# ghnmqdtg/VM-ASR

Measured on AMD Instinct MI355X. Metric: audio clips/sec (train step) 48kHz n_fft=1024, higher is better.
Workload: dtype bf16 (autocast over G; scan/STFT f32; MPD f32/bf16x3 MFMA); 1 GPU; vm_asr_48k_MPD.yaml full train step, DIMS 16 d_state 1 n_fft 1024 clip 122640@48k; per_gpu_batch=4, global_batch=4, parallelism=dp1, execution=hipGraph replay, 2 streams, generator_streams=2

## Files before the change

### include/vmasr_hip.h

```cpp
#ifndef VMASR_HIP_H
#define VMASR_HIP_H

#include <stddef.h>
#include <stdint.h>

#ifdef __cplusplus
extern "C" {
#endif

#define VMASR_ABI_VERSION 1

typedef void *vmasr_stream_t;

enum { VMASR_F32 = 0, VMASR_F16 = 1, VMASR_BF16 = 2 };

enum {
    VMASR_OK = 0,
    VMASR_EINVAL = -1,
    VMASR_EALIGN = -2,
    VMASR_ENOSPACE = -3
};

int vmasr_abi_version(void);
const char *vmasr_last_error(void);
// ... 119 lines not shown
                           int32_t in_features, int32_t out_features, int32_t x_dtype, int32_t y_dtype,
                           vmasr_stream_t stream);
size_t vmasr_small_linear_bwd_workspace(int64_t rows, int32_t in_features, int32_t out_features);
int vmasr_small_linear_bwd(const void *x, const float *w, const void *gy, void *dx, float *dw, float *db,
                           float *ws, int64_t rows, int32_t in_features, int32_t out_features,
                           int32_t x_dtype, int32_t gy_dtype, vmasr_stream_t stream);

int vmasr_spectral_power_iter(const float *W, float *u, float *v, float *ws, int32_t R, int32_t C,
                              int32_t n_iter, float eps, vmasr_stream_t stream);

typedef struct vmasr_spectral_item {
    const float *W;
    float *u, *v, *t, *s;
    int32_t R, C, row_block_start, col_tile_start;
} vmasr_spectral_item;
int vmasr_spectral_power_iter_batched(const vmasr_spectral_item *items, int32_t n, int32_t total_row_blocks,
                                      int32_t total_col_tiles, int64_t weight_bytes, int32_t n_iter, float eps,
                                      float *sigma, vmasr_stream_t stream);

int vmasr_im2col_kx1(const void *x, void *cols, int64_t N, int32_t H, int32_t C, int32_t k, int32_t stride,
                     int32_t pad, int64_t rows_out, int32_t dtype, vmasr_stream_t stream);
int vmasr_im2col_kx1_split(const float *x, void *hi, void *lo, int64_t N, int32_t H, int32_t C, int32_t k, int32_t stride,
                           int32_t pad, int64_t rows_out, vmasr_stream_t stream);
int vmasr_col2im_kx1(const void *dcols, void *dx, int64_t N, int32_t H, int32_t C, int32_t k, int32_t stride,
                     int32_t pad, int32_t dtype, vmasr_stream_t stream);
int vmasr_im2col_kx1_split_multi(const float *const *xs, const int64_t *Ns, const int32_t *Hs, int32_t n, void *hi, void *lo,
                                 int32_t C, int32_t k, int32_t stride, int32_t pad, int64_t rows_out, vmasr_stream_t stream);
int vmasr_im2col_kx1_split3_multi(const float *const *xs, const int64_t *Ns, const int32_t *Hs, int32_t n, void *cat3, int32_t C,
                                  int32_t k, int32_t stride, int32_t pad, int64_t rows_out, vmasr_stream_t stream);
int vmasr_col2im_kx1_multi(const void *dcols, void *const *dxs, const int64_t *Ns, const int32_t *Hs, int32_t n, int32_t C,
                           int32_t k, int32_t stride, int32_t pad, int64_t rows, int32_t dtype, vmasr_stream_t stream);
int vmasr_col2im_kx1_stacked(const void *dcols, void *dx, const int64_t *Ns, const int32_t *Hs, int32_t n, int32_t C, int32_t k, int32_t stride,
                             int32_t pad, int64_t rows, int64_t dx_rows, int32_t dtype, vmasr_stream_t stream);
int vmasr_stack_rows(const void *const *srcs, const int64_t *Ms, int32_t n, void *full, int64_t rows, int64_t row_bytes,
                     vmasr_stream_t stream);


int vmasr_bias_gelu_fwd(float *acc, const float *bias, float *act, int32_t slots, int64_t M, int32_t N, int32_t parts,
                        vmasr_stream_t stream);
int vmasr_weight_prep_split(const float *w, void *out, int32_t n, int32_t N, int32_t K, vmasr_stream_t stream);
int vmasr_weight_transpose(const float *w, void *hi, void *lo, float *out32, int32_t n, int32_t N, int32_t Cin, int32_t k,
                           vmasr_stream_t stream);
int vmasr_sum_parts(const float *parts, float *out, int32_t P, int32_t n, int32_t S, int64_t NK, vmasr_stream_t stream);
int vmasr_gelu_bwd_split(const float *pre, const float *g, void *hi, void *lo, void *cat3, float *db, int32_t slots, int64_t M,
                         int32_t N, vmasr_stream_t stream);
int vmasr_gelu_bwd(const float *pre, const float *g, float *gx, float *db, int32_t slots, int64_t M, int32_t N, vmasr_stream_t stream);

typedef struct vmasr_cg_slot {
    const void *ah, *al;
    const void *bh, *bl;
    float *c0;
    float *c1;
    void *ch, *cl;
    const float *bias;
    int64_t nseq;
    int32_t H;
    int32_t reserved;
} vmasr_cg_slot;
int vmasr_conv_mfma_supported(int32_t Cin, int32_t Cout, int32_t k, int32_t stride);
int vmasr_conv_mfma_supported_launch(int32_t Cin, int32_t Cout, int32_t k, int32_t stride, int32_t n, int64_t rows);
int vmasr_conv_mfma_config(int32_t pass, int32_t Cin, int32_t Cout, int32_t ops, int32_t out[3]);
void vmasr_conv_set_cu_limit(int32_t cus);
int32_t vmasr_conv_get_cu_limit(void);
int vmasr_conv_mfma_fwd(const vmasr_cg_slot *slots, int32_t n, int32_t Cin, int32_t Cout, int32_t k, int32_t stride, int32_t pad,
                        int64_t rows_out, int32_t act, vmasr_stream_t stream);
int vmasr_conv_mfma_dgrad(const vmasr_cg_slot *slots, int32_t n, int32_t Cin, int32_t Cout, int32_t k, int32_t stride, int32_t pad,
                          int64_t rows_in, vmasr_stream_t stream);
int vmasr_conv_f32_fwd(const vmasr_cg_slot *slots, int32_t n, int32_t Cin, int32_t Cout, int32_t k, int32_t stride, int32_t pad,
                       int64_t rows_out, int32_t act, vmasr_stream_t stream);
int vmasr_conv_f32_dgrad(const vmasr_cg_slot *slots, int32_t n, int32_t Cin, int32_t Cout, int32_t k, int32_t stride, int32_t pad,
                         int64_t rows_in, vmasr_stream_t stream);
int vmasr_conv_mfma_wgrad(const vmasr_cg_slot *slots, int32_t n, int32_t Cin, int32_t Cout, int32_t k, int32_t stride, int32_t pad,
                          int32_t splits, vmasr_stream_t stream);
typedef struct vmasr_cg_gelu_bwd {
    const float *pre;
    const signed char *sgn;
    int64_t valid;
    float scale;
    int32_t reserved;
    float *db;
} vmasr_cg_gelu_bwd;
int vmasr_conv_mfma_dgrad_gelu(const vmasr_cg_slot *slots, const vmasr_cg_gelu_bwd *epi, const float *gtok, int32_t n, int32_t Cin, int32_t Cout,
                               int32_t k, int32_t stride, int32_t pad, int64_t rows_in, vmasr_stream_t stream);

int vmasr_wgrad_finish_multi(const float *const *parts, float *const *dws, float *const *dbs, float *const *e1s, float *const *e2s,
                             const int32_t *Ss, const int32_t *Ns, const int32_t *Ks, const int32_t *lds, int32_t n, vmasr_stream_t stream);

int vmasr_linear_f64acc(const float *x, const float *w, const float *bias, float *y, int64_t rows, int32_t out_features,
                        int32_t in_features, vmasr_stream_t stream);

typedef struct vmasr_adamw_item {
    float *p;
    const float *g;
    float *m;
    float *v;
    void *lp;
    int64_t n;
    float weight_decay;
    int32_t vec;
    void *lpt;
    int32_t rows, cols;
} vmasr_adamw_item;
int32_t vmasr_adamw_chunk(void);
int vmasr_adamw_step(const vmasr_adamw_item *items, const int32_t *chunks, int32_t nchunks, int64_t total_elems, const float *lr,
                     const float *step, float beta1, float beta2, float eps, vmasr_stream_t stream);

int32_t vmasr_sn_dot_blocks(void);
int vmasr_sn_stack_fwd(const void *const *weights, const void *const *sigmas, int32_t n, float *out, void *hi, void *lo, int32_t N, int32_t Cin,
                       int32_t k, vmasr_stream_t stream);
int vmasr_sn_stack_bwd(const float *dW, const float *Wn, void *const *gws, const void *const *sigmas, const void *const *us,
                       const void *const *vs, int32_t n, double *partials, int32_t N, int32_t Cin, int32_t k, vmasr_stream_t stream);

int vmasr_conv_post_supported(int32_t C, int32_t k);
int vmasr_conv_post_fwd(const float *x, const float *w, const float *b, float *y, const int64_t *Ms, const int32_t *Hs, int32_t n, int64_t rows,
                        int32_t C, int32_t k, vmasr_stream_t stream);
int vmasr_conv_post_bwd(const float *x, const float *w, const float *gy, float *dx, float *dw, float *db, const int64_t *Ms, const int32_t *Hs,
                        int32_t n, int64_t rows, int32_t C, int32_t k, vmasr_stream_t stream);
int vmasr_conv_post_bwd_gelu(const float *x, const float *w, const float *gy, const float *pre, const void *sgn, const float *gtok,
                             const int64_t *valid, const float *scale, void *gh, void *gl, float *g32, float *dw, float *db, float *dbcol,
                             const int64_t *Ms, const int32_t *Hs, int32_t n, int64_t rows, int32_t C, int32_t k, vmasr_stream_t stream);

int vmasr_conv_first_fwd(const void *const *xs, const int64_t *Ns, const int32_t *Hs, int32_t n, const float *w, const float *b, float *pre,
                         float *act, int64_t rows, vmasr_stream_t stream);
int vmasr_conv_first_bwd(const void *const *xs, const int64_t *Ns, const int32_t *Hs, int32_t n, const float *w, const float *pre,
                         const float *g, float *dcols, float *dw, float *db, int64_t rows, vmasr_stream_t stream);

int32_t vmasr_masked_l1_blocks(void);
int vmasr_masked_l1_fwd(const float *real, const float *gen, void *sgn, double *partials, const int64_t *valid, const float *scale,
                        int32_t n, int64_t rows_r, int64_t rows_g, int32_t N, vmasr_stream_t stream);
int vmasr_masked_l1_bwd(const void *sgn, const float *gout, float *dgen, const int64_t *valid, const float *scale, int32_t n,
                        int64_t rows_g, int32_t N, vmasr_stream_t stream);
int vmasr_masked_l1_bwd_add(const void *sgn, const float *gout, const float *add, float *dgen, const int64_t *valid, const float *scale,
                            int32_t n, int64_t rows_g, int32_t N, vmasr_stream_t stream);
int vmasr_lsgan_fwd(const void *const *xs, const int64_t *ns, const float *targets, int32_t count, float *out, vmasr_stream_t stream);
int vmasr_lsgan_bwd(const void *const *xs, void *const *ds, const int64_t *ns, const float *targets, int32_t count, const float *gout,
                    vmasr_stream_t stream);

#define VMASR_SS2D_PAIRS 1
typedef struct vmasr_ss2d_params {
    int32_t B, D, H, W, dtype, flags;
    const void *x;
    void *xT;
    const float *Wx, *Wdt, *dtb, *Alog, *Ds;
    float *state, *out02, *out13, *y;
    const float *dy;
    float *dyT, *adj, *part;
    void *dx;
    float *dWx, *dWdt, *ddtb, *dAlog, *dDs;
} vmasr_ss2d_params;
int vmasr_ss2d_supported(int32_t d_state, int32_t dt_rank, int32_t d_inner, int32_t H, int32_t W);
size_t vmasr_ss2d_part_floats(int32_t B, int32_t D, int32_t H, int32_t W);
int vmasr_ss2d_fwd(const vmasr_ss2d_params *p, vmasr_stream_t stream);
int vmasr_ss2d_bwd(const vmasr_ss2d_params *p, vmasr_stream_t stream);

typedef struct vmasr_ss2d_deep_params {
    int32_t B, D, H, W, R, dtype;
    const void *x;
    const float *WxT, *Wdt, *dtb, *Alog, *Ds;
    float *xdbl, *y;
    const float *dy;
    float *du;
    void *tp, *tb, *tc;
    float *pg, *g32;
    void *dx, *gpos;
} vmasr_ss2d_deep_params;
int vmasr_ss2d_deep_supported(int32_t d_state, int32_t dt_rank, int32_t d_inner, int32_t H, int32_t W);
// ... 97 lines not shown
int vmasr_dconv1d_dgrad(const float *gy, const float *pre, const float *w, float *dx, void *ws, size_t ws_bytes, int32_t B, int32_t Cin,
                        int32_t Cout, int32_t groups, int64_t L, int32_t k, int32_t stride, int32_t pad, vmasr_stream_t stream);
int vmasr_dconv1d_wgrad(const float *x, const float *gy, const float *pre, float *dw, float *db, void *ws, size_t ws_bytes, int32_t B,
                        int32_t Cin, int32_t Cout, int32_t groups, int64_t L, int32_t k, int32_t stride, int32_t pad, vmasr_stream_t stream);

enum {
    VMASR_K_SSCAN_FWD = 0,
    VMASR_K_SSCAN_FWD_AGG,
    VMASR_K_SSCAN_FWD_CARRY,
    VMASR_K_SSCAN_FWD_APPLY,
    VMASR_K_SSCAN_BWD,
    VMASR_K_SSCAN_BWD_AGG,
    VMASR_K_SSCAN_BWD_CARRY,
    VMASR_K_SSCAN_BWD_APPLY,
    VMASR_K_CROSS_SCAN,
    VMASR_K_CROSS_MERGE,
    VMASR_K_DWCONV_FWD,
    VMASR_K_DWCONV_BWD_A,
    VMASR_K_DWCONV_BWD_B,
    VMASR_K_STFT,
    VMASR_K_ISTFT_FRAMES,
    VMASR_K_ISTFT_OLA,
    VMASR_K_ISTFT_BWD,
    VMASR_K_LN_FWD,
    VMASR_K_LN_BWD,
    VMASR_K_LN_BWD_REDUCE,
    VMASR_K_SMALL_LINEAR_FWD,
    VMASR_K_SMALL_LINEAR_BWD,
    VMASR_K_SMALL_LINEAR_REDUCE,
    VMASR_K_XPROJ_FWD,
    VMASR_K_XPROJ_BWD_A,
    VMASR_K_XPROJ_BWD_B,
    VMASR_K_SPECTRAL,
    VMASR_K_IM2COL,
    VMASR_K_COL2IM,
    VMASR_K_SPLIT_BF16,
    VMASR_K_BIAS_GELU,
    VMASR_K_SS2D_TRANSPOSE,
    VMASR_K_SS2D_FWD_AGG,
    VMASR_K_SS2D_CARRY,
    VMASR_K_SS2D_FWD_APPLY,
    VMASR_K_SS2D_MERGE,
    VMASR_K_SS2D_BWD_AGG,
    VMASR_K_SS2D_BWD_APPLY,
    VMASR_K_SS2D_PRE,
    VMASR_K_LN_GATE,
    VMASR_K_STACK_ROWS,
    VMASR_K_FEAT_L1,
    VMASR_K_ADAMW,
    VMASR_K_CONV_POST,
    VMASR_K_CONV_POST_BWD_GELU,
    VMASR_K_WEIGHT_T,
    VMASR_K_MLP_FWD,
    VMASR_K_MLP_BWD,
    VMASR_K_INPROJ_FWD,
    VMASR_K_INPROJ_BWD,
    VMASR_K_SS2D_DEEP_XPROJ,
    VMASR_K_SS2D_DEEP_FWD,
    VMASR_K_SS2D_DEEP_BWD,
    VMASR_K_SS2D_DEEP_XBWD,
    VMASR_K_OUTPROJ_FWD,
    VMASR_K_OUTPROJ_BWD,
    VMASR_K_STFT_LOSS,
    VMASR_K_CONV_MFMA_FWD,
    VMASR_K_CONV_MFMA_DGRAD,
    VMASR_K_CONV_MFMA_WGRAD,
    VMASR_K_WGRAD_FINISH,
    VMASR_K_SKINNY_LINEAR,
    VMASR_K_METRICS,
    VMASR_K_RESAMPLE_DESIGN,
    VMASR_K_DEGRADE_BATCH,
    VMASR_K_GCONV1D_FWD,
    VMASR_K_GCONV1D_DGRAD,
    VMASR_K_GCONV1D_WGRAD,
    VMASR_K_GCONV1D_WGRAD_REDUCE,
    VMASR_K_STEM1D_FWD,
    VMASR_K_STEM1D_BWD,
    VMASR_K_STEM1D_BWD_REDUCE,
    VMASR_K_DCONV1D_FWD,
    VMASR_K_DCONV1D_DGRAD,
    VMASR_K_DCONV1D_REDUCE,
    VMASR_K_DCONV1D_WGRAD,
    VMASR_K_DCONV1D_WGRAD_REDUCE,
    VMASR_K_RESAMPLE,
    VMASR_K_COUNT
};
void vmasr_set_deterministic(int on);
int vmasr_get_deterministic(void);
int64_t vmasr_det_timeouts(void);
void vmasr_prof_enable(int on);
void vmasr_prof_reset(void);
const char *vmasr_prof_name(int kernel_id);
int vmasr_prof_collect(int kernel_id, int64_t *launches, double *total_ms, double *alg_bytes);
int vmasr_mark_time(uint64_t *dst, vmasr_stream_t stream);

int vmasr_im2col2d_rows(const void *x, void *cols, int32_t B, int32_t C, int32_t H, int32_t W, int32_t kh, int32_t kw, int32_t sh, int32_t sw,
                        int32_t ph, int32_t pw, const int64_t *x_strides, int32_t x_dtype, int32_t cols_dtype, vmasr_stream_t stream);
int vmasr_col2im2d_rows(const void *gcols, void *dx, int32_t B, int32_t C, int32_t H, int32_t W, int32_t kh, int32_t kw, int32_t sh, int32_t sw,
                        int32_t ph, int32_t pw, const int64_t *dx_strides, int32_t cols_dtype, int32_t dx_dtype, vmasr_stream_t stream);
int vmasr_skinny_linear_supported(int64_t rows, int32_t in_f, int32_t out_f);
int vmasr_skinny_linear(const void *x, const float *w, const float *bias, void *y, int64_t rows, int32_t in_f, int32_t out_f,
                        int64_t w_stride_out, int64_t w_stride_in, int32_t x_dtype, int32_t y_dtype, vmasr_stream_t stream);
int vmasr_prof_collect_shapes(int kernel_id, int max_groups, double *group_bytes, int64_t *group_launches, double *group_ms);

#ifdef __cplusplus
}
#endif
#endif
```

### vm_asr_amd/_lib.py

```python
import ctypes
import os

from . import knobs

_HERE = os.path.dirname(os.path.abspath(__file__))
LIB_PATH = knobs.get("VMASR_LIB") or os.path.join(_HERE, "libvmasr_hip.so")

c_i32, c_i64, c_vp, c_sz = ctypes.c_int32, ctypes.c_int64, ctypes.c_void_p, ctypes.c_size_t

F32, F16, BF16 = 0, 1, 2


class SScanParams(ctypes.Structure):
    _fields_ = (
        [(n, c_i32) for n in ("batch", "dim", "seqlen", "dstate", "n_groups", "n_chunks", "dtype",
                              "delta_softplus")]
        + [(n, c_i64) for n in ("A_d_stride", "A_dstate_stride",
                                "B_batch_stride", "B_group_stride", "B_dstate_stride",
                                "C_batch_stride", "C_group_stride", "C_dstate_stride",
                                "u_batch_stride", "u_d_stride", "delta_batch_stride", "delta_d_stride",
                                "out_batch_stride", "out_d_stride")]
        + [(n, c_vp) for n in ("A_ptr", "B_ptr", "C_ptr", "D_ptr", "u_ptr", "delta_ptr",
                               "delta_bias_ptr", "out_ptr", "x_ptr")]
    )


class SScanBwdParams(ctypes.Structure):
    _fields_ = (
        [("f", SScanParams)]
        + [(n, c_i64) for n in ("dout_batch_stride", "dout_d_stride", "du_batch_stride", "du_d_stride",
                                "ddelta_batch_stride", "ddelta_d_stride", "dA_d_stride", "dA_dstate_stride")]
        + [(n, c_vp) for n in ("dout_ptr", "du_ptr", "ddelta_ptr", "dA_ptr", "dB_ptr", "dC_ptr", "dD_ptr",
                               "ddelta_bias_ptr", "ws_ptr")]
        + [("ws_bytes", c_sz)]
    )


class SS2DParams(ctypes.Structure):
    _fields_ = ([(n, c_i32) for n in ("B", "D", "H", "W", "dtype", "flags")]
                + [(n, c_vp) for n in ("x", "xT", "Wx", "Wdt", "dtb", "Alog", "Ds", "state", "out02", "out13", "y",
                                       "dy", "dyT", "adj", "part", "dx", "dWx", "dWdt", "ddtb", "dAlog", "dDs")])


class CgSlot(ctypes.Structure):
    _fields_ = ([(n, c_vp) for n in ("ah", "al", "bh", "bl", "c0", "c1", "ch", "cl", "bias")]
                + [("nseq", c_i64), ("H", c_i32), ("reserved", c_i32)])


class CgGeluBwd(ctypes.Structure):
    _fields_ = [("pre", c_vp), ("sgn", c_vp), ("valid", c_i64), ("scale", ctypes.c_float), ("reserved", c_i32), ("db", c_vp)]


class SS2DDeepParams(ctypes.Structure):
    _fields_ = ([(n, c_i32) for n in ("B", "D", "H", "W", "R", "dtype")]
                + [(n, c_vp) for n in ("x", "WxT", "Wdt", "dtb", "Alog", "Ds", "xdbl", "y", "dy", "du", "tp", "tb", "tc", "pg",
                                       "g32", "dx", "gpos")])


SYMBOLS = {
    "vmasr_abi_version": (ctypes.c_int, []),
    "vmasr_last_error": (ctypes.c_char_p, []),
    "vmasr_sscan_chunk": (ctypes.c_int, []),
    "vmasr_sscan_fwd": (ctypes.c_int, [ctypes.POINTER(SScanParams), c_vp]),
    "vmasr_sscan_bwd_workspace": (c_sz, [ctypes.POINTER(SScanBwdParams)]),
    "vmasr_sscan_bwd": (ctypes.c_int, [ctypes.POINTER(SScanBwdParams), c_vp]),
    "vmasr_sscan_tune": (None, [ctypes.c_int, ctypes.c_int]),
    "vmasr_layer_norm_fwd": (ctypes.c_int, [c_vp, c_vp, c_vp, c_vp, c_vp, c_vp, c_i32, c_i32, ctypes.c_float, c_i32, c_i32, c_vp]),
    "vmasr_layer_norm_bwd_workspace": (c_sz, [c_i32, c_i32]),
    "vmasr_layer_norm_bwd": (ctypes.c_int, [c_vp, c_vp, c_vp, c_vp, c_vp, c_vp, c_vp, c_vp, c_vp, c_i32, c_i32, c_i32, c_i32, c_vp]),
    "vmasr_layer_norm_bwd_res": (ctypes.c_int, [c_vp, c_vp, c_vp, c_vp, c_vp, c_vp, c_vp, c_vp, c_vp, c_vp, c_i32, c_i32, c_i32, c_i32, c_vp]),
    "vmasr_layer_norm_bwd_blocks": (c_i32, [c_i32, c_i32]),
    "vmasr_layer_norm_bwd_reduce_multi": (ctypes.c_int, [c_vp, c_vp, c_vp, c_vp, c_vp, c_i32, c_vp]),
    "vmasr_mlp_supported": (ctypes.c_int, [c_i32, c_i32]),
    "vmasr_mlp_fwd": (ctypes.c_int, [c_vp, c_vp, c_vp, ctypes.c_float, c_vp, c_vp, c_vp, c_vp, c_vp, c_i32, c_vp, c_i64, c_i32, c_i32, c_vp]),
    "vmasr_mlp_bwd": (ctypes.c_int, [c_vp, c_vp, c_vp, c_vp, ctypes.c_float, c_vp, c_vp, c_vp, c_vp, c_vp, c_i32,
                                     c_vp, c_vp, c_vp, c_vp, c_vp, c_vp, c_vp, c_i64, c_i32, c_i32, c_vp]),
    "vmasr_stft_loss_blocks": (c_i32, []),
    "vmasr_stft_loss_fwd": (ctypes.c_int, [c_vp, c_vp, c_vp, c_vp, c_i64, c_vp, c_vp, c_vp]),
    "vmasr_stft_loss_bwd": (ctypes.c_int, [c_vp, c_vp, c_vp, c_vp, c_i64, c_vp, c_vp, c_vp, c_vp, c_vp, c_vp]),
    "vmasr_outproj_supported": (ctypes.c_int, [c_i32, c_i32]),
    "vmasr_outproj_fwd": (ctypes.c_int, [c_vp, c_vp, c_vp, c_vp, c_i32, c_vp, c_i64, c_i32, c_i32, c_vp]),
    "vmasr_outproj_bwd": (ctypes.c_int, [c_vp, c_vp, c_vp, c_i32, c_vp, c_vp, c_i64, c_i32, c_i32, c_vp]),
    "vmasr_inproj_supported": (ctypes.c_int, [c_i32, c_i32, c_i64]),
    "vmasr_inproj_fwd": (ctypes.c_int, [c_vp, c_vp, c_vp, ctypes.c_float, c_vp, c_vp, c_vp, c_i64, c_i32, c_i32, c_i32, c_vp]),
    "vmasr_inproj_bwd": (ctypes.c_int, [c_vp, c_vp, c_vp, ctypes.c_float, c_vp, c_vp, c_vp, c_vp, c_vp, c_vp, c_vp, c_vp, c_vp,
                                        c_i64, c_i32, c_i32, c_i32, c_vp]),
    "vmasr_small_linear_supported": (ctypes.c_int, [c_i32, c_i32]),
    "vmasr_small_linear_fwd": (ctypes.c_int, [c_vp, c_vp, c_vp, c_vp, c_i64, c_i32, c_i32, c_i32, c_i32, c_vp]),
    "vmasr_small_linear_bwd_workspace": (c_sz, [c_i64, c_i32, c_i32]),
    "vmasr_small_linear_bwd": (ctypes.c_int, [c_vp, c_vp, c_vp, c_vp, c_vp, c_vp, c_vp, c_i64, c_i32, c_i32, c_i32, c_i32, c_vp]),
    "vmasr_cross_scan_cvt": (ctypes.c_int, [c_vp, c_vp, c_i32, c_i32, c_i32, c_i32, c_i32, c_i32, c_vp]),
    "vmasr_cross_merge_cvt": (ctypes.c_int, [c_vp, c_vp, c_i32, c_i32, c_i32, c_i32, c_i32, c_i32, c_vp]),
    "vmasr_xproj_supported": (ctypes.c_int, [c_i32, c_i32, c_i32]),
    "vmasr_xproj_fwd": (ctypes.c_int, [c_vp] * 7 + [c_i32] * 7 + [c_vp]),
    "vmasr_xproj_bwd": (ctypes.c_int, [c_vp] * 12 + [c_i32] * 7 + [c_vp]),
    "vmasr_xproj_n_supported": (ctypes.c_int, [c_i32, c_i32, c_i32]),
    "vmasr_xproj_n_ws_floats": (c_sz, [c_i32, c_i32, c_i32, c_i32]),
    "vmasr_xproj_n_fwd": (ctypes.c_int, [c_vp] * 7 + [c_i32] * 7 + [c_vp]),
    "vmasr_xproj_n_bwd": (ctypes.c_int, [c_vp] * 12 + [c_i32] * 7 + [c_vp]),
    "vmasr_spectral_power_iter": (ctypes.c_int, [c_vp, c_vp, c_vp, c_vp, c_i32, c_i32, c_i32, ctypes.c_float, c_vp]),
    "vmasr_spectral_power_iter_batched": (ctypes.c_int, [c_vp, c_i32, c_i32, c_i32, c_i64, c_i32, ctypes.c_float, c_vp, c_vp]),
    "vmasr_im2col_kx1": (ctypes.c_int, [c_vp, c_vp, c_i64, c_i32, c_i32, c_i32, c_i32, c_i32, c_i64, c_i32, c_vp]),
    "vmasr_im2col_kx1_split": (ctypes.c_int, [c_vp, c_vp, c_vp, c_i64, c_i32, c_i32, c_i32, c_i32, c_i32, c_i64, c_vp]),
    "vmasr_im2col_kx1_split3_multi": (ctypes.c_int, [c_vp, c_vp, c_vp, c_i32, c_vp, c_i32, c_i32, c_i32, c_i32, c_i64, c_vp]),
    "vmasr_col2im_kx1": (ctypes.c_int, [c_vp, c_vp, c_i64, c_i32, c_i32, c_i32, c_i32, c_i32, c_i32, c_vp]),
    "vmasr_im2col_kx1_split_multi": (ctypes.c_int, [c_vp, c_vp, c_vp, c_i32, c_vp, c_vp, c_i32, c_i32, c_i32, c_i32, c_i64, c_vp]),
    "vmasr_col2im_kx1_multi": (ctypes.c_int, [c_vp, c_vp, c_vp, c_vp, c_i32, c_i32, c_i32, c_i32, c_i32, c_i64, c_i32, c_vp]),
    "vmasr_col2im_kx1_stacked": (ctypes.c_int, [c_vp, c_vp, c_vp, c_vp, c_i32, c_i32, c_i32, c_i32, c_i32, c_i64, c_i64, c_i32, c_vp]),
    "vmasr_stack_rows": (ctypes.c_int, [c_vp, c_vp, c_i32, c_vp, c_i64, c_i64, c_vp]),
    "vmasr_split_bf16": (ctypes.c_int, [c_vp, c_vp, c_vp, c_i64, c_vp]),
    "vmasr_bias_gelu_fwd": (ctypes.c_int, [c_vp, c_vp, c_vp, c_i32, c_i64, c_i32, c_i32, c_vp]),
    "vmasr_gelu_bwd": (ctypes.c_int, [c_vp, c_vp, c_vp, c_vp, c_i32, c_i64, c_i32, c_vp]),
    "vmasr_sn_dot_blocks": (c_i32, []),
    "vmasr_sn_stack_fwd": (ctypes.c_int, [c_vp, c_vp, c_i32, c_vp, c_vp, c_vp, c_i32, c_i32, c_i32, c_vp]),
    "vmasr_sn_stack_bwd": (ctypes.c_int, [c_vp, c_vp, c_vp, c_vp, c_vp, c_vp, c_i32, c_vp, c_i32, c_i32, c_i32, c_vp]),
    "vmasr_conv_post_supported": (ctypes.c_int, [c_i32, c_i32]),
    "vmasr_conv_post_fwd": (ctypes.c_int, [c_vp, c_vp, c_vp, c_vp, c_vp, c_vp, c_i32, c_i64, c_i32, c_i32, c_vp]),
    "vmasr_conv_post_bwd": (ctypes.c_int, [c_vp, c_vp, c_vp, c_vp, c_vp, c_vp, c_vp, c_vp, c_i32, c_i64, c_i32, c_i32, c_vp]),
    "vmasr_conv_post_bwd_gelu": (ctypes.c_int, [c_vp] * 16 + [c_i32, c_i64, c_i32, c_i32, c_vp]),
    "vmasr_conv_first_fwd": (ctypes.c_int, [c_vp, c_vp, c_vp, c_i32, c_vp, c_vp, c_vp, c_vp, c_i64, c_vp]),
    "vmasr_conv_first_bwd": (ctypes.c_int, [c_vp, c_vp, c_vp, c_i32, c_vp, c_vp, c_vp, c_vp, c_vp, c_vp, c_i64, c_vp]),
    "vmasr_adamw_chunk": (c_i32, []),
    "vmasr_adamw_step": (ctypes.c_int, [c_vp, c_vp, c_i32, c_i64, c_vp, c_vp, ctypes.c_float, ctypes.c_float, ctypes.c_float, c_vp]),
    "vmasr_masked_l1_blocks": (c_i32, []),
    "vmasr_masked_l1_fwd": (ctypes.c_int, [c_vp, c_vp, c_vp, c_vp, c_vp, c_vp, c_i32, c_i64, c_i64, c_i32, c_vp]),
    "vmasr_masked_l1_bwd": (ctypes.c_int, [c_vp, c_vp, c_vp, c_vp, c_vp, c_i32, c_i64, c_i32, c_vp]),
    "vmasr_lsgan_fwd": (ctypes.c_int, [c_vp, c_vp, c_vp, c_i32, c_vp, c_vp]),
    "vmasr_lsgan_bwd": (ctypes.c_int, [c_vp, c_vp, c_vp, c_vp, c_i32, c_vp, c_vp]),
    "vmasr_masked_l1_bwd_add": (ctypes.c_int, [c_vp, c_vp, c_vp, c_vp, c_vp, c_vp, c_i32, c_i64, c_i32, c_vp]),
    "vmasr_sum_parts": (ctypes.c_int, [c_vp, c_vp, c_i32, c_i32, c_i32, c_i64, c_vp]),
    "vmasr_weight_prep_split": (ctypes.c_int, [c_vp, c_vp, c_i32, c_i32, c_i32, c_vp]),
    "vmasr_weight_transpose": (ctypes.c_int, [c_vp, c_vp, c_vp, c_vp, c_i32, c_i32, c_i32, c_i32, c_vp]),
    "vmasr_gelu_bwd_split": (ctypes.c_int, [c_vp, c_vp, c_vp, c_vp, c_vp, c_vp, c_i32, c_i64, c_i32, c_vp]),
    "vmasr_conv_mfma_supported": (ctypes.c_int, [c_i32, c_i32, c_i32, c_i32]),
    "vmasr_conv_mfma_supported_launch": (ctypes.c_int, [c_i32, c_i32, c_i32, c_i32, c_i32, ctypes.c_int64]),
    "vmasr_conv_mfma_config": (ctypes.c_int, [c_i32, c_i32, c_i32, c_i32, ctypes.POINTER(c_i32)]),
    "vmasr_mark_time": (ctypes.c_int, [c_vp, c_vp]),
    "vmasr_im2col2d_rows": (ctypes.c_int, [c_vp, c_vp] + [c_i32] * 10 + [c_vp, c_i32, c_i32, c_vp]),
    "vmasr_col2im2d_rows": (ctypes.c_int, [c_vp, c_vp] + [c_i32] * 10 + [c_vp, c_i32, c_i32, c_vp]),
    "vmasr_skinny_linear_supported": (ctypes.c_int, [c_i64, c_i32, c_i32]),
    "vmasr_skinny_linear": (ctypes.c_int, [c_vp, c_vp, c_vp, c_vp, c_i64, c_i32, c_i32, c_i64, c_i64, c_i32, c_i32, c_vp]),
    "vmasr_conv_set_cu_limit": (None, [c_i32]),
    "vmasr_conv_get_cu_limit": (c_i32, []),
    "vmasr_conv_mfma_fwd": (ctypes.c_int, [ctypes.POINTER(CgSlot), c_i32, c_i32, c_i32, c_i32, c_i32, c_i32, c_i64, c_i32, c_vp]),
    "vmasr_conv_mfma_dgrad": (ctypes.c_int, [ctypes.POINTER(CgSlot), c_i32, c_i32, c_i32, c_i32, c_i32, c_i32, c_i64, c_vp]),
    "vmasr_conv_f32_fwd": (ctypes.c_int, [ctypes.POINTER(CgSlot), c_i32, c_i32, c_i32, c_i32, c_i32, c_i32, c_i64, c_i32, c_vp]),
    "vmasr_conv_f32_dgrad": (ctypes.c_int, [ctypes.POINTER(CgSlot), c_i32, c_i32, c_i32, c_i32, c_i32, c_i32, c_i64, c_vp]),
    "vmasr_conv_mfma_wgrad": (ctypes.c_int, [ctypes.POINTER(CgSlot), c_i32, c_i32, c_i32, c_i32, c_i32, c_i32, c_i32, c_vp]),
    "vmasr_conv_mfma_dgrad_gelu": (ctypes.c_int, [ctypes.POINTER(CgSlot), ctypes.POINTER(CgGeluBwd), c_vp, c_i32, c_i32, c_i32, c_i32, c_i32,
                                                  c_i32, c_i64, c_vp]),
    "vmasr_wgrad_finish_multi": (ctypes.c_int, [c_vp, c_vp, c_vp, c_vp, c_vp, c_vp, c_vp, c_vp, c_vp, c_i32, c_vp]),
    "vmasr_linear_f64acc": (ctypes.c_int, [c_vp, c_vp, c_vp, c_vp, c_i64, c_i32, c_i32, c_vp]),
    "vmasr_ss2d_glue_supported": (ctypes.c_int, [c_i32, c_i32, c_i32]),
    "vmasr_ss2d_pre_fwd": (ctypes.c_int, [c_vp, c_vp, c_vp, c_i32, c_i32, c_i32, c_i32, c_vp]),
    "vmasr_ss2d_pre_bwd": (ctypes.c_int, [c_vp, c_vp, c_vp, c_vp, c_i32, c_i32, c_i32, c_i32, c_vp]),
    "vmasr_ln_gate_fwd": (ctypes.c_int, [c_vp] * 7 + [c_i32, c_i32, c_i32, ctypes.c_float, c_i32, c_vp]),
    "vmasr_ln_gate_bwd": (ctypes.c_int, [c_vp] * 11 + [c_i32, c_i32, c_i32, c_i32, c_vp]),
    "vmasr_ln_gate_bwd_workspace": (c_i64, [c_i32, c_i32, c_i32, c_i32]),
    "vmasr_ln_gate_bwd_ws": (ctypes.c_int, [c_vp] * 12 + [c_i32, c_i32, c_i32, c_i32, c_vp]),
    "vmasr_ln_gate_pair_supported": (ctypes.c_int, [c_i32, c_i32, c_i32]),
    "vmasr_ln_gate_pair_fwd": (ctypes.c_int, [c_vp] * 8 + [c_i32, c_i32, c_i32, c_i32, ctypes.c_float, c_i32, c_vp]),
    "vmasr_ln_gate_pair_bwd": (ctypes.c_int, [c_vp] * 13 + [c_i32, c_i32, c_i32, c_i32, c_i32, c_vp]),
    "vmasr_ss2d_supported": (ctypes.c_int, [c_i32] * 5),
    "vmasr_ss2d_part_floats": (c_sz, [c_i32] * 4),
    "vmasr_ss2d_fwd": (ctypes.c_int, [ctypes.POINTER(SS2DParams), c_vp]),
    "vmasr_ss2d_bwd": (ctypes.c_int, [ctypes.POINTER(SS2DParams), c_vp]),
    "vmasr_ss2d_deep_supported": (ctypes.c_int, [c_i32] * 5),
    "vmasr_ss2d_deep_waves_per_row": (c_i32, [c_i32, c_i32]),
    "vmasr_ss2d_deep_fwd": (ctypes.c_int, [ctypes.POINTER(SS2DDeepParams), c_vp]),
    "vmasr_ss2d_deep_bwd": (ctypes.c_int, [ctypes.POINTER(SS2DDeepParams), c_vp]),
    "vmasr_set_deterministic": (None, [ctypes.c_int]),
    "vmasr_get_deterministic": (ctypes.c_int, []),
    "vmasr_det_timeouts": (ctypes.c_int64, []),
    "vmasr_prof_enable": (None, [ctypes.c_int]),
    "vmasr_prof_reset": (None, []),
    "vmasr_prof_name": (ctypes.c_char_p, [ctypes.c_int]),
    "vmasr_prof_collect": (ctypes.c_int, [ctypes.c_int, ctypes.POINTER(ctypes.c_int64),
                                          ctypes.POINTER(ctypes.c_double), ctypes.POINTER(ctypes.c_double)]),
    "vmasr_prof_collect_shapes": (ctypes.c_int, [ctypes.c_int, ctypes.c_int, ctypes.POINTER(ctypes.c_double), ctypes.POINTER(ctypes.c_int64),
                                                 ctypes.POINTER(ctypes.c_double)]),
    "vmasr_cross_scan": (ctypes.c_int, [c_vp, c_vp, c_i32, c_i32, c_i32, c_i32, c_i32, c_vp]),
    "vmasr_cross_merge": (ctypes.c_int, [c_vp, c_vp, c_i32, c_i32, c_i32, c_i32, c_i32, c_vp]),
    "vmasr_dwconv_silu_fwd": (ctypes.c_int, [c_vp, c_vp, c_vp, c_vp, c_i32, c_i32, c_i32, c_i32, c_i32, c_vp]),
    "vmasr_dwconv_silu_bwd": (ctypes.c_int, [c_vp, c_vp, c_vp, c_vp, c_vp, c_vp, c_vp, c_vp,
                                             c_i32, c_i32, c_i32, c_i32, c_i32, c_vp]),
    "vmasr_stft": (ctypes.c_int, [c_vp, c_vp, c_vp, c_i32, c_i32, c_i32, c_i32, c_i32, c_i32, c_i32, c_vp]),
    "vmasr_stft_bwd_workspace": (c_sz, [c_i32, c_i32, c_i32, c_i32]),
    "vmasr_stft_bwd": (ctypes.c_int, [c_vp, c_vp, c_vp, c_i32, c_i32, c_i32, c_i32, c_i32, c_i32, c_vp, c_sz, c_vp]),
    "vmasr_istft_workspace": (c_sz, [c_i32, c_i32, c_i32, c_i32]),
    "vmasr_istft": (ctypes.c_int, [c_vp, c_vp, c_vp, c_i32, c_i32, c_i32, c_i32, c_i32, c_vp, c_sz, c_vp]),
    "vmasr_istft_bwd": (ctypes.c_int, [c_vp, c_vp, c_vp, c_vp, c_vp, c_i32, c_i32, c_i32, c_i32, c_i32, c_vp]),
    "vmasr_metrics_workspace": (c_sz, [c_i32, c_i32, c_i32, c_i32]),
    "vmasr_metrics": (ctypes.c_int, [c_vp, c_vp, c_vp, c_vp, c_vp, c_i32, c_i32, c_i32, c_i32, c_vp, c_sz, c_vp]),
    "vmasr_gconv1d_supported": (ctypes.c_int, [c_i32] * 5),
    "vmasr_gconv1d_supported_launch": (ctypes.c_int, [c_i32] * 7 + [c_i64]),
    "vmasr_gconv1d_wgrad_workspace": (c_sz, [c_i32] * 7 + [c_i64]),
    "vmasr_gconv1d_fwd": (ctypes.c_int, [c_vp] * 5 + [c_i32] * 4 + [c_i64] + [c_i32] * 4 + [c_vp]),
    "vmasr_gconv1d_dgrad": (ctypes.c_int, [c_vp] * 4 + [c_i32] * 4 + [c_i64] + [c_i32] * 3 + [c_vp]),
    "vmasr_gconv1d_wgrad": (ctypes.c_int, [c_vp] * 6 + [c_sz] + [c_i32] * 4 + [c_i64] + [c_i32] * 3 + [c_vp]),
    "vmasr_dconv1d_pos_tile": (c_i32, []),
    "vmasr_dconv1d_m_tile": (c_i32, []),
    "vmasr_dconv1d_k_chunk": (c_i32, []),
    "vmasr_dconv1d_max_taps": (c_i32, []),
    "vmasr_dconv1d_supported": (ctypes.c_int, [c_i32] * 5),
    "vmasr_dconv1d_supported_launch": (ctypes.c_int, [c_i32] * 7 + [c_i64]),
    "vmasr_dconv1d_fwd_slabs": (c_i32, [c_i32] * 7 + [c_i64]),
    "vmasr_dconv1d_fwd_workspace": (c_sz, [c_i32] * 7 + [c_i64]),
    "vmasr_dconv1d_dgrad_workspace": (c_sz, [c_i32] * 7 + [c_i64]),
    "vmasr_dconv1d_wgrad_workspace": (c_sz, [c_i32] * 7 + [c_i64]),
    "vmasr_dconv1d_fwd": (ctypes.c_int, [c_vp] * 6 + [c_sz] + [c_i32] * 4 + [c_i64] + [c_i32] * 4 + [c_vp]),
    "vmasr_dconv1d_dgrad": (ctypes.c_int, [c_vp] * 5 + [c_sz] + [c_i32] * 4 + [c_i64] + [c_i32] * 3 + [c_vp]),
    "vmasr_dconv1d_wgrad": (ctypes.c_int, [c_vp] * 6 + [c_sz] + [c_i32] * 4 + [c_i64] + [c_i32] * 3 + [c_vp]),
    "vmasr_stem1d_time_tile": (c_i32, []),
    "vmasr_stem1d_channel_group": (c_i32, []),
    "vmasr_stem1d_supported": (ctypes.c_int, [c_i32] * 4),
    "vmasr_stem1d_supported_launch": (ctypes.c_int, [c_i32] * 5 + [c_i64]),
    "vmasr_stem1d_bwd_workspace": (c_sz, [c_i32] * 5 + [c_i64]),
    "vmasr_stem1d_fwd": (ctypes.c_int, [c_vp] * 4 + [c_i32] * 2 + [c_i64] + [c_i32] * 4 + [c_vp]),
    "vmasr_stem1d_bwd": (ctypes.c_int, [c_vp] * 8 + [c_sz] + [c_i32] * 2 + [c_i64] + [c_i32] * 4 + [c_vp]),
    "vmasr_stem1d_fm_supported_launch": (ctypes.c_int, [c_i32] * 5 + [c_i64]),
    "vmasr_stem1d_fm_workspace": (c_sz, [c_i32] * 5 + [c_i64]),
    "vmasr_stem1d_fm_fwd": (ctypes.c_int, [c_vp] * 6 + [c_sz] + [c_i32] * 2 + [c_i64] + [c_i32] * 3 + [c_vp]),
    "vmasr_stem1d_fm_bwd": (ctypes.c_int, [c_vp] * 6 + [ctypes.c_float] + [c_vp] + [c_i32] * 2 + [c_i64] + [c_i32] * 3 + [c_vp]),
    "vmasr_resample_poly": (ctypes.c_int, [c_vp, c_vp, c_vp, c_i32, c_i64, c_i64, c_i32, c_i32, c_i32, c_vp]),
    "vmasr_resample_design_workspace": (c_sz, [c_i32]),
    "vmasr_resample_design": (ctypes.c_int, [c_vp, c_i32, c_i32, c_i32, c_vp, c_sz, c_vp]),
    "vmasr_degrade_batch_workspace": (c_sz, [c_vp, c_i32]),
# ... 22 lines not shown
        knobs.warn_undeclared()
        _lib = l
    return _lib


def check(code, what):
    if code != 0:
        msg = lib().vmasr_last_error().decode() or "unknown error"
        raise RuntimeError(f"{what} failed ({code}): {msg}")


def torch_dtype_code(dt):
    import torch
    try:
        return {torch.float32: F32, torch.float16: F16, torch.bfloat16: BF16}[dt]
    except KeyError:
        raise RuntimeError(f"unsupported dtype {dt}: expected float32 / float16 / bfloat16")


def det_mode():
    if knobs.get("VMASR_DETERMINISTIC"):
        return True
    try:
        return bool(lib().vmasr_get_deterministic())
    except (OSError, RuntimeError, AttributeError):
        return False


def current_stream(device):
    import torch
    return ctypes.c_void_p(torch.cuda.current_stream(device).cuda_stream)


def ptr(t):
    return None if t is None else ctypes.c_void_p(t.data_ptr())


def call(fn, *args, device=None):
    import torch
    what = fn.__name__[len("vmasr_"):]
    conv = list(args)
    for i, a in enumerate(conv):
        t = type(a)
        if t is int or t is float or a is None:
            continue
        if isinstance(a, torch.Tensor):
            if not a.is_cuda:
                require_cuda(what, a)
            if device is None:
                device = a.device
            conv[i] = ctypes.c_void_p(a.data_ptr())
        elif isinstance(a, ctypes.Structure):
            conv[i] = ctypes.byref(a)
    if device is None:
        raise RuntimeError(f"{what}: no tensor argument and no device= to launch on")
    with torch.cuda.device(device):
        check(fn(*conv, current_stream(device)), what)


def require_cuda(name, *tensors):
    if not all(t.is_cuda for t in tensors):
        raise RuntimeError(f"{name}: expected a CUDA (HIP) tensor; vm_asr_amd has no CPU path")


def bf16_autocast():
    import torch
    return torch.is_autocast_enabled("cuda") and torch.get_autocast_dtype("cuda") == torch.bfloat16


def autocast_dtype(x):
    import torch
    return torch.get_autocast_dtype("cuda") if torch.is_autocast_enabled("cuda") else x.dtype


def f32c(t, shape):
    return t.detach().float().reshape(shape).contiguous()


def rows2d(t, width):
    t2 = t.reshape(-1, width)
    return t2 if t2.is_contiguous() else t2.contiguous()


K_COUNT = 78


def zeros_f32(device, *shapes):
    import torch
    sizes = [0 if sh is None else -(-int(torch.Size(sh).numel()) // 4) * 4 for sh in shapes]
    flat = torch.zeros(max(1, sum(sizes)), dtype=torch.float32, device=device)
    out, off = [], 0
    for sh, n in zip(shapes, sizes):
        out.append(None if sh is None else flat[off:off + torch.Size(sh).numel()].view(sh))
        off += n
    return out


def prof_enable(on=True):
    lib().vmasr_prof_enable(int(bool(on)))


def prof_reset():
    lib().vmasr_prof_reset()


def prof_collect():
    l = lib()
    out = {}
    for k in range(K_COUNT):
        n, ms, by = ctypes.c_int64(0), ctypes.c_double(0.0), ctypes.c_double(0.0)
        check(l.vmasr_prof_collect(k, ctypes.byref(n), ctypes.byref(ms), ctypes.byref(by)), "prof_collect")
        if n.value:
            out[l.vmasr_prof_name(k).decode()] = dict(launches=n.value, ms=ms.value, alg_bytes=by.value)
    return out


def prof_collect_shapes(name, max_groups=16):
    l = lib()
    for k in range(K_COUNT):
        if l.vmasr_prof_name(k).decode() == name:
            by, n, ms = (ctypes.c_double * max_groups)(), (ctypes.c_int64 * max_groups)(), (ctypes.c_double * max_groups)()
            ng = l.vmasr_prof_collect_shapes(k, max_groups, by, n, ms)
            if ng < 0:
                raise RuntimeError(f"prof_collect_shapes failed ({ng})")
            return [dict(alg_bytes_per_launch=by[i], launches=n[i], ms=ms[i]) for i in range(ng)]
    raise KeyError(name)
```

### vm_asr_amd/convgemm.py

```python
import ctypes

import torch

from . import _lib
from .mpd_ops import need as _need, sum_parts


def supported(Cin, Cout, k, stride):
    return bool(_lib.lib().vmasr_conv_mfma_supported(int(Cin), int(Cout), int(k), int(stride)))


def config(what, Cin, Cout, f32=False):
    out = (ctypes.c_int32 * 3)()
    _lib.check(_lib.lib().vmasr_conv_mfma_config(("fwd", "dgrad", "wgrad").index(what), int(Cin), int(Cout), int(bool(f32)), out), "conv_mfma_config")
    return tuple(out)


_LIMIT = {"cus": 0, "min_channels": 0}


class cu_limit:

    def __init__(self, cus, min_channels=0):
        self.new = {"cus": int(cus or 0), "min_channels": int(min_channels or 0)}

    def __enter__(self):
        self.prev = dict(_LIMIT)
        _LIMIT.update(self.new)
        return self

    def __exit__(self, *exc):
        _LIMIT.update(self.prev)
        _lib.lib().vmasr_conv_set_cu_limit(0)
        return False


def _apply_limit(Cin, Cout):
    lim = _LIMIT["cus"] if max(Cin, Cout) >= _LIMIT["min_channels"] else 0
    _lib.lib().vmasr_conv_set_cu_limit(lim)


def _slots(geom, **operands):
    sl = (_lib.CgSlot * len(geom))()
    steps = [(f, t.data_ptr(), t.stride(0) * t.element_size()) for f, t in operands.items() if t is not None]
    for i, (nseq, H) in enumerate(geom):
        for f, base, step in steps:
            setattr(sl[i], f, base + i * step)
        sl[i].nseq, sl[i].H = int(nseq), int(H)
    return sl


def _ptr(t, i, step):
    return ctypes.c_void_p(t.data_ptr() + i * step) if t is not None else None


def out_positions(H, k, stride, pad):
    return (H + 2 * pad - k) // stride + 1


def _fwd(fn, xh, xl, wh, wl, bias, geom, k, stride, pad, rows_out, act, want_pair):
    _need(xh, xl, wh, wl, bias)
    (n, _, Cin), Cout, dev = xh.shape, wh.shape[1], xh.device
    pre = torch.empty((n, rows_out, Cout), dtype=torch.float32, device=dev)
    y = torch.empty_like(pre) if act else None
    yh = torch.empty((n, rows_out, Cout), dtype=torch.bfloat16, device=dev) if act and want_pair else None
    yl = torch.empty_like(yh) if yh is not None else None
    sl = _slots(geom, ah=xh, al=xl, bh=wh, bl=wl, c0=pre, c1=y, ch=yh, cl=yl, bias=bias)
    _apply_limit(Cin, Cout)
    _lib.call(fn, sl, n, Cin, Cout, k, stride, pad, rows_out, int(bool(act)), device=dev)
    return pre, y, yh, yl


def _dgrad(fn, gh, gl, wth, wtl, geom, k, stride, pad, rows_in):
    _need(gh, gl, wth, wtl)
    (n, _, Cout), Cin, dev = gh.shape, wth.shape[1], gh.device
    dx = torch.empty((n, rows_in, Cin), dtype=torch.float32, device=dev)
    sl = _slots(geom, ah=gh, al=gl, bh=wth, bl=wtl, c0=dx)
    _apply_limit(Cin, Cout)
    _lib.call(fn, sl, n, Cin, Cout, k, stride, pad, rows_in, device=dev)
    return dx


def conv_fwd(xh, xl, wh, wl, bias, geom, k, stride, pad, rows_out, act=True, want_pair=True):
    return _fwd(_lib.lib().vmasr_conv_mfma_fwd, xh, xl, wh, wl, bias, geom, k, stride, pad, rows_out, act, want_pair)


def conv_dgrad(gh, gl, wth, wtl, geom, k, stride, pad, rows_in):
    return _dgrad(_lib.lib().vmasr_conv_mfma_dgrad, gh, gl, wth, wtl, geom, k, stride, pad, rows_in)


def conv_fwd_f32(x, w, bias, geom, k, stride, pad, rows_out, act=True, want_pair=True):
    assert x.dtype == torch.float32 and w.dtype == torch.float32
    return _fwd(_lib.lib().vmasr_conv_f32_fwd, x, None, w, None, bias, geom, k, stride, pad, rows_out, act, want_pair)


def conv_dgrad_f32(g, wt, geom, k, stride, pad, rows_in):
    assert g.dtype == torch.float32 and wt.dtype == torch.float32
    return _dgrad(_lib.lib().vmasr_conv_f32_dgrad, g, None, wt, None, geom, k, stride, pad, rows_in)


def conv_dgrad_gelu(gh, gl, wth, wtl, geom, k, stride, pad, rows_in, pre, want_f32=False, want_pair=True, sgn=None, gtok=None,
                    scale=None, valid=None, db=None):
    _need(gh, gl, wth, wtl, pre, sgn, gtok, db)
    assert db is None or (db.shape == (gh.shape[0], wth.shape[1]) and db.dtype == torch.float32)
    (n, _, Cout), Cin, dev = gh.shape, wth.shape[1], gh.device
    assert pre.shape == (n, rows_in, Cin) and pre.dtype == torch.float32 and (want_f32 or want_pair)
    assert sgn is None or (sgn.shape == pre.shape and sgn.dtype == torch.int8 and gtok is not None and gtok.dtype == torch.float32)
    g32 = torch.empty((n, rows_in, Cin), dtype=torch.float32, device=dev) if want_f32 else None
    oh = torch.empty((n, rows_in, Cin), dtype=torch.bfloat16, device=dev) if want_pair else None
    ol = torch.empty_like(oh) if want_pair else None
    sl = _slots(geom, ah=gh, al=gl, bh=wth, bl=wtl, c0=g32, ch=oh, cl=ol)
    ep = (_lib.CgGeluBwd * n)()
    for i in range(n):
        ep[i].pre = _ptr(pre, i, rows_in * Cin * 4)
        ep[i].sgn = _ptr(sgn, i, rows_in * Cin)
        ep[i].valid = int(valid[i]) if (sgn is not None and valid is not None) else 0
        ep[i].scale = float(scale[i]) if (sgn is not None and scale is not None) else 0.0
        ep[i].db = _ptr(db, i, Cin * 4)
    _apply_limit(Cin, Cout)
    _lib.call(_lib.lib().vmasr_conv_mfma_dgrad_gelu, sl, ep, gtok if sgn is not None else None, n, Cin, Cout, k, stride, pad, rows_in,
              device=dev)
    return g32, ((oh, ol) if want_pair else None)


def wgrad_splits(n, Cin, Cout, k, M):
    if Cin % 256 == 0 and Cout % 256 == 0:
        return 1
    T = 128
    tiles = n * (Cout // T) * (k * Cin // T)
    s = 1
    while tiles * s < 768 and s < 16 and M // (2 * s) >= 1024:
        s *= 2
    return s


def conv_wgrad(gh, gl, xh, xl, geom, k, stride, pad, splits=None):
    _need(gh, gl, xh, xl)
    (n, _, Cout), Cin, dev = gh.shape, xh.shape[2], gh.device
    if splits is None:
        M = max(nseq * out_positions(H, k, stride, pad) for nseq, H in geom)
        splits = wgrad_splits(n, Cin, Cout, k, M)
    parts = torch.empty((n, splits, Cout, k * Cin), dtype=torch.float32, device=dev)
    sl = _slots(geom, ah=gh, al=gl, bh=xh, bl=xl, c0=parts)
    _apply_limit(Cin, Cout)
    _lib.call(_lib.lib().vmasr_conv_mfma_wgrad, sl, n, Cin, Cout, k, stride, pad, splits, device=dev)
    if splits == 1:
        return parts.view(n, Cout, k * Cin)
    return sum_parts(parts, 1, n, splits, (Cout, k * Cin))
```

### vm_asr_amd/csrc/api.hip

```cpp
#include "common.h"

#include <mutex>
#include <vector>

namespace vmasr {
namespace {
thread_local char g_err[512] = "";

struct Rec {
    int kid;
    hipEvent_t e0, e1;
    double bytes;
};
std::mutex g_mu;
std::vector<Rec> g_recs;
std::vector<hipEvent_t> g_pool;
thread_local Rec g_open{-1, nullptr, nullptr, 0.0};

hipEvent_t take_event() {
    if (!g_pool.empty()) {
        hipEvent_t e = g_pool.back();
        g_pool.pop_back();
        return e;
    }
    hipEvent_t e = nullptr;
    (void)hipEventCreate(&e);
    return e;
}

const char *kNames[VMASR_K_COUNT] = {
    "sscan_fwd", "sscan_fwd_agg", "sscan_fwd_carry", "sscan_fwd_apply", "sscan_bwd", "sscan_bwd_agg",
    "sscan_bwd_carry", "sscan_bwd_apply", "cross_scan", "cross_merge", "dwconv_silu_fwd", "dwconv_silu_bwd_a",
    "dwconv_silu_bwd_b", "stft", "istft_frames", "istft_ola", "istft_bwd", "layer_norm_fwd", "layer_norm_bwd",
    "layer_norm_bwd_reduce", "small_linear_fwd", "small_linear_bwd", "small_linear_reduce",
    "xproj_fwd", "xproj_bwd_a", "xproj_bwd_b", "spectral_power_iter", "im2col_kx1", "col2im_kx1", "split_bf16", "bias_gelu",
    "ss2d_transpose", "ss2d_fwd_agg", "ss2d_carry", "ss2d_fwd_apply", "ss2d_merge", "ss2d_bwd_agg", "ss2d_bwd_apply",
    "ss2d_pre", "ln_gate", "stack_rows", "feat_l1", "adamw", "conv_post", "conv_post_bwd_gelu", "weight_transpose", "mlp_fwd", "mlp_bwd", "inproj_fwd", "inproj_bwd",
    "ss2d_deep_xproj", "ss2d_deep_fwd", "ss2d_deep_bwd", "ss2d_deep_xbwd", "outproj_fwd", "outproj_bwd", "stft_loss",
    "conv_mfma_fwd", "conv_mfma_dgrad", "conv_mfma_wgrad", "wgrad_finish", "skinny_linear", "metrics", "resample_design", "degrade_batch",
    "gconv1d_fwd", "gconv1d_dgrad", "gconv1d_wgrad", "gconv1d_wgrad_reduce",
    "stem1d_fwd", "stem1d_bwd", "stem1d_bwd_reduce",
    "dconv1d_fwd", "dconv1d_dgrad", "dconv1d_reduce", "dconv1d_wgrad", "dconv1d_wgrad_reduce", "resample_poly"};
}

bool g_prof_on = false;
static bool g_det_on = false;
constexpr int kMaxDev = 16;
static unsigned *g_det_buf[kMaxDev] = {};

unsigned *det_ticket(int kid) {
    if (!g_det_on || kid < 0 || kid >= VMASR_K_COUNT) return nullptr;
    int dev = 0;
    if (hipGetDevice(&dev) != hipSuccess || dev < 0 || dev >= kMaxDev || g_det_buf[dev] == nullptr) {
        set_error("deterministic mode: no ticket buffer for device %d (vmasr_set_deterministic(1) must run before the first launch)", dev);
        return nullptr;
    }
    return g_det_buf[dev] + kid;
}
static int det_prepare() {
    int n = 0, cur = 0;
    if (hipGetDeviceCount(&n) != hipSuccess || n <= 0) return 0;
    (void)hipGetDevice(&cur);
    int rc = 0;
    for (int d = 0; d < n && d < kMaxDev; ++d) {
        if (g_det_buf[d]) continue;
        if (hipSetDevice(d) != hipSuccess || hipMalloc(reinterpret_cast<void **>(&g_det_buf[d]), 2 * VMASR_K_COUNT * sizeof(unsigned)) != hipSuccess ||
            hipMemset(g_det_buf[d], 0, 2 * VMASR_K_COUNT * sizeof(unsigned)) != hipSuccess || hipDeviceSynchronize() != hipSuccess) {
            g_det_buf[d] = nullptr;
            set_error("deterministic mode: cannot allocate the ticket buffer of device %d (switch the mode on outside a stream capture)", d);
            rc = VMASR_EINVAL;
        }
    }
    (void)hipSetDevice(cur);
    return rc;
}
void det_set(bool on) { g_det_on = on; }
bool det_get() { return g_det_on; }

void set_error(const char *fmt, ...) {
    va_list ap;
    va_start(ap, fmt);
    vsnprintf(g_err, sizeof(g_err), fmt, ap);
    va_end(ap);
}

void prof_begin(int kid, hipStream_t st, double bytes) {
    std::lock_guard<std::mutex> lk(g_mu);
    g_open = Rec{kid, take_event(), take_event(), bytes};
    (void)hipEventRecord(g_open.e0, st);
}

void prof_end(hipStream_t st) {
    std::lock_guard<std::mutex> lk(g_mu);
    if (g_open.kid < 0) return;
    (void)hipEventRecord(g_open.e1, st);
    g_recs.push_back(g_open);
    g_open.kid = -1;
}
}

using namespace vmasr;

VMASR_EXPORT int vmasr_abi_version(void) { return VMASR_ABI_VERSION; }
VMASR_EXPORT const char *vmasr_last_error(void) { return g_err; }

VMASR_EXPORT void vmasr_prof_enable(int on) { g_prof_on = on != 0; }

VMASR_EXPORT void vmasr_set_deterministic(int on) {
    if (on && vmasr::det_prepare() != 0) return;
    vmasr::det_set(on != 0);
}
VMASR_EXPORT int64_t vmasr_det_timeouts(void) {
    int64_t total = 0;
    int cur = 0;
    (void)hipGetDevice(&cur);
    for (int d = 0; d < vmasr::kMaxDev; ++d) {
        if (!vmasr::g_det_buf[d]) continue;
        unsigned host[VMASR_K_COUNT];
        if (hipSetDevice(d) != hipSuccess || hipDeviceSynchronize() != hipSuccess ||
            hipMemcpy(host, vmasr::g_det_buf[d] + VMASR_K_COUNT, sizeof(host), hipMemcpyDeviceToHost) != hipSuccess) { total = -1; break; }
        for (unsigned v : host) total += v;
    }
    (void)hipSetDevice(cur);
    return total;
}
// ... 68 lines not shown
```

### vm_asr_amd/csrc/convgemm.hip

```cpp
#include <algorithm>
#include <cstdlib>
#include <type_traits>

#include "common.h"

namespace vmasr {
namespace {

typedef __bf16 bf16x8 __attribute__((ext_vector_type(8)));
typedef float f32x16 __attribute__((ext_vector_type(16)));
typedef float f32x4 __attribute__((ext_vector_type(4)));
typedef unsigned u32x4 __attribute__((ext_vector_type(4)));
typedef __attribute__((address_space(1))) const void *cg_gptr;
typedef __attribute__((address_space(3))) void *cg_lptr;
__device__ uint4 cg_zero_page[4];

constexpr int CG_BM = 128, CG_BN = 128, CG_BK = 32;
constexpr int CG_TILE = CG_BM * CG_BK * 2;
constexpr int CG_STAGE = 4 * CG_TILE;
constexpr int CG_MAXP = 24;

struct CgProb {
    const bf16_t *ah, *al, *bh, *bl;
    float *c0, *c1;
    bf16_t *ch, *cl;
    const float *bias;
    int M, Q;
    int HA;
    int HC;
    int hq_mul, hq_add;
    int crow_mul, crow_add;
    int ntaps, tap0, tap_step, dstep;
    int tile_start, mtiles;
    int zero_rows;
    float fscale;
    int fvalid;
    float *db;
};

struct CgParams {
    CgProb prob[CG_MAXP];
    int nprob, ntiles_n, total_tiles;
    int CA;
    int NB;
    int KB;
    const float *gtok;
};
static_assert(sizeof(CgParams) <= 4096, "CgParams is passed by value as the kernel's argument block");

__device__ __forceinline__ int cg_swz(const int row) { return (0 - (row >> 2)) & 3; }
__device__ __forceinline__ int cg_off(const int row, const int chunk) { return row * 64 + ((chunk ^ cg_swz(row)) << 4); }

__device__ __forceinline__ float cg_gelu(float x) { return 0.5f * x * (1.f + erff(x * 0.70710678118654752f)); }
__device__ __forceinline__ float cg_gelu_grad(float x) {
    return 0.5f * (1.f + erff(x * 0.70710678118654752f)) + x * 0.3989422804014327f * __expf(-0.5f * x * x);
}

__device__ __forceinline__ f32x16 cg_mfma(const bf16x8 a, const bf16x8 b, const f32x16 c) {
    return __builtin_amdgcn_mfma_f32_32x32x16_bf16(a, b, c, 0, 0, 0);
}

template <int BM, int BN, int WM, int WN, int EPI, int MF, int OPS = 0>
__global__ __launch_bounds__(64 * WM * WN, 2) void conv_mfma_nt_kernel(const CgParams P) {
    static_assert(OPS == 0 || MF == 32, "the f32 form uses the 32-row fragment layout");
    constexpr bool ACT = EPI == 1;
    constexpr int NT = 64 * WM * WN;
    constexpr int WTM = BM / WM, WTN = BN / WN;
    constexpr int TI = WTM / MF, TJ = WTN / MF;
    constexpr int TILE_A = BM * 64, TILE_B = BN * 64;
    constexpr int STAGE = 2 * TILE_A + 2 * TILE_B;
    constexpr int RPP = NT / 4;
    constexpr int PA = BM / RPP, PB = (BN + RPP - 1) / RPP;
    constexpr bool B_PART = BN < RPP;
    static_assert(BM % RPP == 0 && (BN % RPP == 0 || (B_PART && BN % 16 == 0)) && BM % 128 == 0, "tile / thread geometry");
    extern __shared__ __attribute__((aligned(16))) unsigned char smem[];
    int *crow_tab = reinterpret_cast<int *>(smem + 2 * STAGE);

    const int tid = threadIdx.x, lane = tid & 63, wave = tid >> 6;
    const int wm = wave / WN, wn = wave % WN, lr = lane & 31, lh = lane >> 5;

#pragma unroll 1
    for (int tile = blockIdx.x; tile < P.total_tiles; tile += gridDim.x) {
    const int t = xcd_remap(tile, P.total_tiles);
    int pi = 0;
#pragma unroll 1
    for (int i = 1; i < P.nprob; ++i) pi = (t >= P.prob[i].tile_start) ? i : pi;
    const CgProb &pr = P.prob[pi];
    const int local = t - pr.tile_start;
    const int nt = local % P.ntiles_n, mt = local / P.ntiles_n;
    const int m0 = mt * BM, n0 = nt * BN;
    const int M = pr.M, Q = pr.Q, HA = pr.HA, CA = P.CA, NB = P.NB;
    constexpr int UPK = OPS ? 64 : 32;
    const int LDA = OPS ? 2 * CA : CA;
    const int KB = OPS ? 2 * P.KB : P.KB;

    if (tid < BM) {
        const int m = m0 + tid;
        int cr = -1;
        if (m < M) {
            const int seq = m / Q, q = m - seq * Q;
            cr = seq * pr.HC + q * pr.crow_mul + pr.crow_add;
        } else if (m < pr.zero_rows) {
            cr = m;
        }
        crow_tab[tid] = cr;
    }

    const int srow = tid >> 2, chunk = (tid & 3) ^ cg_swz(srow);
    int a_base[PA], a_hq[PA];
    bool a_ok[PA];
#pragma unroll
    for (int i = 0; i < PA; ++i) {
        const int m = m0 + srow + RPP * i;
        a_ok[i] = m < M;
        const int mm = a_ok[i] ? m : 0;
        const int seq = mm / Q, q = mm - seq * Q;
        a_base[i] = seq * HA;
        a_hq[i] = q * pr.hq_mul + pr.hq_add;
    }
    const bf16_t *bsrc_h[PB], *bsrc_l[PB];
#pragma unroll
    for (int i = 0; i < PB; ++i) {
        const size_t o = (size_t)(n0 + ((B_PART && srow >= BN) ? 0 : srow + RPP * i)) * KB + chunk * 8;
        bsrc_h[i] = pr.bh + o;
        bsrc_l[i] = pr.bl + o;
    }
    const int cpk = CA / CG_BK;
    const int nk = (m0 < M) ? pr.ntaps * cpk : 0;
    const int wbase = wave * 16 * 64;
    const bf16_t *zp = reinterpret_cast<const bf16_t *>(cg_zero_page);

#define CG_DMA(src, dst) __builtin_amdgcn_global_load_lds((cg_gptr)(src), (cg_lptr)(dst), 16, 0, 0)
    auto stage_tile = [&](const int kt, const int buf) {
        const int j = kt / cpk, c0 = (kt - j * cpk) * UPK;
        const int koff = (pr.tap0 + j * pr.tap_step) * LDA + c0;
        unsigned char *d = smem + buf * STAGE + wbase;
#pragma unroll
        for (int i = 0; i < PA; ++i) {
            const int pos = a_hq[i] + j * pr.dstep;
// ... 34 lines not shown
                f32x4 a0[TI], a1[TI], b0[TJ], b1[TJ];
#pragma unroll
                for (int i = 0; i < TI; ++i) {
                    const int oa = cg_off(wm * WTM + i * 32 + lr, ks * 2 + lh);
                    a0[i] = *reinterpret_cast<const f32x4 *>(s + oa);
                    a1[i] = *reinterpret_cast<const f32x4 *>(s + TILE_A + oa);
                }
#pragma unroll
                for (int j = 0; j < TJ; ++j) {
                    const int ob = cg_off(wn * WTN + j * 32 + lr, ks * 2 + lh);
                    b0[j] = *reinterpret_cast<const f32x4 *>(s + 2 * TILE_A + ob);
                    b1[j] = *reinterpret_cast<const f32x4 *>(s + 2 * TILE_A + TILE_B + ob);
                }
#pragma unroll
                for (int i = 0; i < TI; ++i)
#pragma unroll
                    for (int j = 0; j < TJ; ++j) {
#pragma unroll
                        for (int e = 0; e < 4; ++e) acc[i][j] = __builtin_amdgcn_mfma_f32_32x32x2f32(a0[i][e], b0[j][e], acc[i][j], 0, 0, 0);
#pragma unroll
                        for (int e = 0; e < 4; ++e) acc[i][j] = __builtin_amdgcn_mfma_f32_32x32x2f32(a1[i][e], b1[j][e], acc[i][j], 0, 0, 0);
                    }
            }
        } else if constexpr (MF == 32) {
#pragma unroll
            for (int ks = 0; ks < 2; ++ks) {
                bf16x8 ah[TI], al[TI], bh[TJ], bl[TJ];
#pragma unroll
                for (int i = 0; i < TI; ++i) {
                    const int oa = cg_off(wm * WTM + i * 32 + lr, ks * 2 + lh);
                    ah[i] = *reinterpret_cast<const bf16x8 *>(s + oa);
                    al[i] = *reinterpret_cast<const bf16x8 *>(s + TILE_A + oa);
                }
#pragma unroll
                for (int j = 0; j < TJ; ++j) {
                    const int ob = cg_off(wn * WTN + j * 32 + lr, ks * 2 + lh);
                    bh[j] = *reinterpret_cast<const bf16x8 *>(s + 2 * TILE_A + ob);
                    bl[j] = *reinterpret_cast<const bf16x8 *>(s + 2 * TILE_A + TILE_B + ob);
                }
#pragma unroll
                for (int i = 0; i < TI; ++i)
#pragma unroll
                    for (int j = 0; j < TJ; ++j) {
                        acc[i][j] = cg_mfma(al[i], bh[j], acc[i][j]);
                        acc[i][j] = cg_mfma(ah[i], bl[j], acc[i][j]);
                        acc[i][j] = cg_mfma(ah[i], bh[j], acc[i][j]);
                    }
            }
        } else {
            const int r16 = lane & 15, c16 = lane >> 4;
            bf16x8 bh[TJ], bl[TJ];
#pragma unroll
            for (int j = 0; j < TJ; ++j) {
                const int ob = cg_off(wn * WTN + j * 16 + r16, c16);
                bh[j] = *reinterpret_cast<const bf16x8 *>(s + 2 * TILE_A + ob);
                bl[j] = *reinterpret_cast<const bf16x8 *>(s + 2 * TILE_A + TILE_B + ob);
            }
#pragma unroll
            for (int i = 0; i < TI; ++i) {
                const int oa = cg_off(wm * WTM + i * 16 + r16, c16);
                const bf16x8 ah = *reinterpret_cast<const bf16x8 *>(s + oa);
                const bf16x8 al = *reinterpret_cast<const bf16x8 *>(s + TILE_A + oa);
#pragma unroll
                for (int j = 0; j < TJ; ++j) {
                    acc[i][j] = __builtin_amdgcn_mfma_f32_16x16x32_bf16(al, bh[j], acc[i][j], 0, 0, 0);
                    acc[i][j] = __builtin_amdgcn_mfma_f32_16x16x32_bf16(ah, bl[j], acc[i][j], 0, 0, 0);
                    acc[i][j] = __builtin_amdgcn_mfma_f32_16x16x32_bf16(ah, bh[j], acc[i][j], 0, 0, 0);
                }
            }
        }
        asm volatile("s_waitcnt vmcnt(0)" ::: "memory");
        __syncthreads();
    }
#undef CG_DMA

    float *ct = reinterpret_cast<float *>(smem);
    static_assert(128 * BN * 4 <= 2 * STAGE, "epilogue tile must fit the staging buffers");
    constexpr int C4 = BN / 4;
    constexpr int RPI = NT / C4;
    const int c4 = tid % C4;
    float4 bias4 = make_float4(0.f, 0.f, 0.f, 0.f);
    float4 dbs = make_float4(0.f, 0.f, 0.f, 0.f);
    float gs = 0.f;
    if constexpr (EPI == 2) {
        if (pr.c1 && P.gtok) gs = P.gtok[0] * pr.fscale;
    } else {
        if (pr.bias) bias4 = *reinterpret_cast<const float4 *>(pr.bias + n0 + 4 * c4);
    }
#pragma unroll 1
    for (int h = 0; h < BM / 128; ++h) {
        if (h > 0) __syncthreads();
        if ((wm * WTM) / 128 == h) {
#pragma unroll
            for (int i = 0; i < TI; ++i)
#pragma unroll
                for (int j = 0; j < TJ; ++j)
#pragma unroll
                    for (int r = 0; r < NR; ++r) {
                        if constexpr (MF == 32)
                            ct[((wm * WTM) % 128 + i * 32 + (r & 3) + 8 * (r >> 2) + 4 * lh) * BN + wn * WTN + j * 32 + lr] = acc[i][j][r];
                        else
                            ct[((wm * WTM) % 128 + i * 16 + 4 * (lane >> 4) + r) * BN + wn * WTN + j * 16 + (lane & 15)] = acc[i][j][r];
                    }
        }
        __syncthreads();
        static_assert(128 % RPI == 0, "epilogue geometry");
#pragma unroll 4
        for (int it = 0; it < 128 / RPI; ++it) {
            const int row = it * RPI + tid / C4;
            const int cr = crow_tab[h * 128 + row];
            if (cr < 0) continue;
            const bool live = m0 + h * 128 + row < M;
            const size_t o = (size_t)cr * NB + n0 + 4 * c4;
            float4 v = *reinterpret_cast<const float4 *>(ct + row * BN + 4 * c4);
            if (live) { v.x += bias4.x; v.y += bias4.y; v.z += bias4.z; v.w += bias4.w; }
            else v = make_float4(0.f, 0.f, 0.f, 0.f);
            if constexpr (EPI == 2) {
                if (live) {
                    if (gs != 0.f && cr < pr.fvalid) {
                        const char4 c = *reinterpret_cast<const char4 *>(reinterpret_cast<const signed char *>(pr.c1) + o);
                        v.x = fmaf(gs, (float)c.x, v.x); v.y = fmaf(gs, (float)c.y, v.y); v.z = fmaf(gs, (float)c.z, v.z); v.w = fmaf(gs, (float)c.w, v.w);
                    }
                    const float4 p = *reinterpret_cast<const float4 *>(pr.bias + o);
                    v.x *= cg_gelu_grad(p.x); v.y *= cg_gelu_grad(p.y); v.z *= cg_gelu_grad(p.z); v.w *= cg_gelu_grad(p.w);
                    dbs.x += v.x; dbs.y += v.y; dbs.z += v.z; dbs.w += v.w;
                }
                if (pr.c0) *reinterpret_cast<float4 *>(pr.c0 + o) = v;
                if (pr.ch) {
                    union { uint2 raw; bf16_t e[4]; } hh, ll;
                    const float yy[4] = {v.x, v.y, v.z, v.w};
#pragma unroll
                    for (int e = 0; e < 4; ++e) {
                        hh.e[e] = (bf16_t)yy[e];
                        ll.e[e] = (bf16_t)(yy[e] - (float)hh.e[e]);
                    }
                    *reinterpret_cast<uint2 *>(pr.ch + o) = hh.raw;
                    *reinterpret_cast<uint2 *>(pr.cl + o) = ll.raw;
                }
                continue;
            }
            *reinterpret_cast<float4 *>(pr.c0 + o) = v;
            if constexpr (ACT) {
                float4 y = make_float4(0.f, 0.f, 0.f, 0.f);
                if (live) y = make_float4(cg_gelu(v.x), cg_gelu(v.y), cg_gelu(v.z), cg_gelu(v.w));
                if (pr.c1) *reinterpret_cast<float4 *>(pr.c1 + o) = y;
                if (pr.ch) {
                    union { uint2 raw; bf16_t e[4]; } hh, ll;
                    const float yy[4] = {y.x, y.y, y.z, y.w};
#pragma unroll
                    for (int e = 0; e < 4; ++e) {
                        hh.e[e] = (bf16_t)yy[e];
                        ll.e[e] = (bf16_t)(yy[e] - (float)hh.e[e]);
                    }
                    *reinterpret_cast<uint2 *>(pr.ch + o) = hh.raw;
                    *reinterpret_cast<uint2 *>(pr.cl + o) = ll.raw;
                }
            }
        }
    }
    if constexpr (EPI == 2) {
        if (pr.db) {
            __syncthreads();
            *reinterpret_cast<float4 *>(ct + (tid / C4) * BN + 4 * c4) = dbs;
            __syncthreads();
            if (tid < BN) {
                float t = 0.f;
#pragma unroll
                for (int q = 0; q < RPI; ++q) t += ct[q * BN + tid];
                atomicAdd(pr.db + n0 + tid, t);
            }
        }
    }
    __syncthreads();
    }
}

typedef __bf16 bf16x4 __attribute__((ext_vector_type(4)));
typedef __attribute__((address_space(3))) bf16x4 lds_bf16x4;

constexpr int CW_BR = 32;

struct CwProb {
    const bf16_t *gh, *gl, *xh, *xl;
    float *dw;
    int M, Q, H;
    int mchunk;
};
struct CwParams {
    CwProb prob[8];
    int nslots, splits, tiles_co, tiles_kc, Cin, Cout, k, stride, pad;
};

template <int ROWB>
__device__ __forceinline__ int cw_off(const int row, const int ch) {
    if constexpr (ROWB == 64) return row * 64 + (ch << 4);
    else return row * ROWB + ((ch ^ (((row & 3) << 2) | ((row >> 2) & 3))) << 4);
}

template <int ROWB, int MF>
__device__ __forceinline__ bf16x8 cw_frag(const unsigned char *tile, const int ks, const int colbase, const int lane) {
    const int g = lane >> 4, q = (lane & 15) >> 2, p = lane & 3;
    const int ch = (MF == 32 ? ((colbase + 16 * (g & 1)) >> 3) : (colbase >> 3)) + (p >> 1);
    const int r0 = (MF == 32 ? ks * 16 + 8 * (g >> 1) : 8 * g) + q;
    const bf16x4 lo = __builtin_amdgcn_ds_read_tr16_b64_v4bf16((lds_bf16x4 *)(tile + cw_off<ROWB>(r0, ch) + 8 * (p & 1)));
    const bf16x4 hi = __builtin_amdgcn_ds_read_tr16_b64_v4bf16((lds_bf16x4 *)(tile + cw_off<ROWB>(r0 + 4, ch) + 8 * (p & 1)));
    return __builtin_shufflevector(lo, hi, 0, 1, 2, 3, 4, 5, 6, 7);
}

template <int BCO, int BKC, int WM, int WN, int MF>
__global__ __launch_bounds__(64 * WM * WN, 2) void conv_mfma_wgrad_kernel(const CwParams P) {
    constexpr int NT = 64 * WM * WN;
    constexpr int WTM = BCO / WM, WTN = BKC / WN, TI = WTM / MF, TJ = WTN / MF;
    using acc_t = typename std::conditional<MF == 32, f32x16, f32x4>::type;
    constexpr int NR = MF == 32 ? 16 : 4;
    constexpr int RBG = BCO * 2, RBX = BKC * 2;
    constexpr int TILE_G = CW_BR * RBG, TILE_X = CW_BR * RBX;
    constexpr int STAGE = 2 * TILE_G + 2 * TILE_X;
    constexpr int CG = BCO / 8, CX = BKC / 8;
    constexpr int PG = CW_BR * CG / NT, PX = (CW_BR * CX + NT - 1) / NT;
    constexpr bool MID_STORE = MF == 16 && BCO * BKC >= 65536;
    constexpr bool X_PART = CW_BR * CX < NT;
    static_assert(PG >= 1 && (CW_BR * CG) % NT == 0 && (X_PART || (CW_BR * CX) % NT == 0), "staging geometry");
    extern __shared__ __attribute__((aligned(16))) unsigned char smem[];
    const int tid = threadIdx.x, lane = tid & 63, wave = tid >> 6;
    const int wm = wave / WN, wn = wave % WN, lr = lane & 31, lh = lane >> 5;

    const int per_slot = P.splits * P.tiles_co * P.tiles_kc;
#pragma unroll 1
    for (int tile = blockIdx.x; tile < P.nslots * per_slot; tile += gridDim.x) {
    const int t = xcd_remap(tile, P.nslots * per_slot);
    const int slot = t / per_slot;
    int rem = t - slot * per_slot;
    const int split = rem / (P.tiles_co * P.tiles_kc);
    rem -= split * (P.tiles_co * P.tiles_kc);
    const int tco = rem / P.tiles_kc, tkc = rem - tco * P.tiles_kc;
    const CwProb &pr = P.prob[slot];
    const int Cin = P.Cin, Cout = P.Cout;
    const int co0 = tco * BCO, kc0 = tkc * BKC;
    const int tap = kc0 / Cin, c0 = kc0 - tap * Cin;
    const int mbeg = split * pr.mchunk, mend = min(pr.M, mbeg + pr.mchunk);
    const int nk = mend > mbeg ? (mend - mbeg + CW_BR - 1) / CW_BR : 0;

    int g_row[PG], g_ch[PG], g_m[PG];
    int x_row[PX], x_ch[PX], x_m[PX], x_seq[PX], x_q[PX];
#pragma unroll
    for (int i = 0; i < PG; ++i) {
        const int idx = tid + i * NT;
        g_row[i] = idx / CG; g_ch[i] = idx % CG;
        g_m[i] = mbeg + g_row[i];
    }
#pragma unroll
    for (int i = 0; i < PX; ++i) {
        const int idx = tid + i * NT;
// ... 84 lines not shown
                    }
            }
        } else {
            bf16x8 bh[TJ], bl[TJ];
#pragma unroll
            for (int j = 0; j < TJ; ++j) {
                bh[j] = cw_frag<RBX, 16>(s + 2 * TILE_G, 0, wn * WTN + j * 16, lane);
                bl[j] = cw_frag<RBX, 16>(s + 2 * TILE_G + TILE_X, 0, wn * WTN + j * 16, lane);
            }
#pragma unroll
            for (int i = 0; i < TI; ++i) {
                if (MID_STORE && i == TI / 2 && more) CW_STORE(buf ^ 1);
                const bf16x8 ah = cw_frag<RBG, 16>(s, 0, wm * WTM + i * 16, lane);
                const bf16x8 al = cw_frag<RBG, 16>(s + TILE_G, 0, wm * WTM + i * 16, lane);
#pragma unroll
                for (int j = 0; j < TJ; ++j) {
                    acc[i][j] = __builtin_amdgcn_mfma_f32_16x16x32_bf16(al, bh[j], acc[i][j], 0, 0, 0);
                    acc[i][j] = __builtin_amdgcn_mfma_f32_16x16x32_bf16(ah, bl[j], acc[i][j], 0, 0, 0);
                    acc[i][j] = __builtin_amdgcn_mfma_f32_16x16x32_bf16(ah, bh[j], acc[i][j], 0, 0, 0);
                }
            }
        }
        if (!MID_STORE && more) CW_STORE(buf ^ 1);
        __syncthreads();
    }
#undef CW_LOAD
#undef CW_STORE

    const int KC = P.k * Cin;
    float *dw = pr.dw + (size_t)split * Cout * KC;
#pragma unroll
    for (int i = 0; i < TI; ++i)
#pragma unroll
        for (int j = 0; j < TJ; ++j) {
            const int col = kc0 + wn * WTN + j * MF + (MF == 32 ? lr : (lane & 15));
#pragma unroll
            for (int r = 0; r < NR; ++r) {
                const int row = co0 + wm * WTM + i * MF + (MF == 32 ? (r & 3) + 8 * (r >> 2) + 4 * lh : 4 * (lane >> 4) + r);
                dw[(size_t)row * KC + col] = acc[i][j][r];
            }
        }
    __syncthreads();
    }
}

}
}

using namespace vmasr;

namespace {

int g_cg_cu_limit = 0;

int cg_grid(int tiles, size_t smem) {
    if (g_cg_cu_limit <= 0) return tiles;
    const int per_cu = std::max(1, (int)((160 * 1024) / std::max<size_t>(smem, 1)));
    static const int slack = [] { const char *e = getenv("VMASR_CONV_CU_SLACK"); return e ? atoi(e) : 24; }();
    const int cap = std::min(256, g_cg_cu_limit + slack) * per_cu;
    const int rounds = (tiles + cap - 1) / cap;
    const int g = ((tiles + rounds - 1) / rounds + 7) / 8 * 8;
    return std::min(tiles, std::min(g, cap));
}

template <int BM, int BN, int WM, int WN, int MF, int OPS = 0>
int cg_launch_cfg(CgParams &P, int epi, hipStream_t st, int kid, double bytes) {
    int tiles = 0;
    P.ntiles_n = P.NB / BN;
    for (int i = 0; i < P.nprob; ++i) {
        P.prob[i].tile_start = tiles;
        P.prob[i].mtiles = (std::max(P.prob[i].M, P.prob[i].zero_rows) + BM - 1) / BM;
        tiles += P.prob[i].mtiles * P.ntiles_n;
    }
    P.total_tiles = tiles;
    if (tiles == 0) return 0;
    constexpr size_t smem = 2 * (2 * BM * 64 + 2 * BN * 64) + BM * sizeof(int);
    constexpr bool HAS_EPI2 = BN >= 128 && OPS == 0;
    static bool attr_done = false;
    if (!attr_done && smem > 65536) {
        (void)hipFuncSetAttribute(reinterpret_cast<const void *>(&conv_mfma_nt_kernel<BM, BN, WM, WN, 1, MF, OPS>), hipFuncAttributeMaxDynamicSharedMemorySize, (int)smem);
        (void)hipFuncSetAttribute(reinterpret_cast<const void *>(&conv_mfma_nt_kernel<BM, BN, WM, WN, 0, MF, OPS>), hipFuncAttributeMaxDynamicSharedMemorySize, (int)smem);
        if constexpr (HAS_EPI2)
            (void)hipFuncSetAttribute(reinterpret_cast<const void *>(&conv_mfma_nt_kernel<BM, BN, WM, WN, 2, MF, OPS>), hipFuncAttributeMaxDynamicSharedMemorySize, (int)smem);
        attr_done = true;
    }
    if (epi == 1) {
        VMASR_LAUNCH(kid, bytes, (conv_mfma_nt_kernel<BM, BN, WM, WN, 1, MF, OPS>), dim3(cg_grid(tiles, smem)), dim3(64 * WM * WN), smem, st, P);
    } else if (epi == 2) {
        if constexpr (HAS_EPI2) {
            VMASR_LAUNCH(kid, bytes, (conv_mfma_nt_kernel<BM, BN, WM, WN, 2, MF, OPS>), dim3(cg_grid(tiles, smem)), dim3(64 * WM * WN), smem, st, P);
        } else {
            set_error("conv_mfma: no fused activation backward for this tile");
            return VMASR_EINVAL;
        }
    } else {
        VMASR_LAUNCH(kid, bytes, (conv_mfma_nt_kernel<BM, BN, WM, WN, 0, MF, OPS>), dim3(cg_grid(tiles, smem)), dim3(64 * WM * WN), smem, st, P);
    }
    return check_launch("conv_mfma");
}

int env_conv_tile() {
    static const int v = [] { const char *e = getenv("VMASR_CONV_TILE"); return e ? atoi(e) : 0; }();
    return v;
}
int env_conv_mfma() {
    static const int v = [] { const char *e = getenv("VMASR_CONV_MFMA"); return e ? atoi(e) : 16; }();
    return v;
}

struct CgConfig {
    int BM, BN, MF;
};
enum { CG_PASS_FWD = 0, CG_PASS_DGRAD = 1, CG_PASS_WGRAD = 2 };

CgConfig cg_config_nt(int NB, int CA, int ops, bool fwd) {
    if (ops) {
        static const int tile = [] { const char *e = getenv("VMASR_CONV_F32_TILE"); return e ? atoi(e) : 128; }();
        if (!fwd) return {256, 32, 32};
        return tile == 256 ? CgConfig{256, 128, 32} : CgConfig{128, 128, 32};
    }
    const int forced = env_conv_tile();
    const int mf = env_conv_mfma() == 16 ? 16 : 32;
    if (NB % 256 == 0 && forced != 128) return {256, 256, mf};
    if (NB % 128 == 0 && CA == 32 && forced != 128) return {256, 128, 16};
    if (NB == 32) return {256, 32, 16};
    return {128, 128, mf};
}

CgConfig cg_config_wgrad(int Cin, int Cout) {
    if (Cout % 256 == 0 && Cin % 256 == 0 && env_conv_tile() != 128) return {256, 256, 16};
    if (Cin == 32) return {128, 32, 16};
    return {128, 128, env_conv_mfma() == 32 ? 32 : 16};
}

CgConfig cg_config(int pass, int Cin, int Cout, int ops) {
    if (pass == CG_PASS_WGRAD) return cg_config_wgrad(Cin, Cout);
    return pass == CG_PASS_FWD ? cg_config_nt(Cout, Cin, ops, true) : cg_config_nt(Cin, Cout, ops, false);
}

int cg_launch(CgParams &P, int epi, hipStream_t st, int kid, double bytes, int ops = 0, bool fwd = true) {
    const CgConfig c = cg_config_nt(P.NB, P.CA, ops, fwd);
    const int key = c.BM * 1000000 + c.BN * 1000 + c.MF;
    if (ops) {
        switch (key) {
            case 256128032: return cg_launch_cfg<256, 128, 4, 2, 32, 1>(P, epi, st, kid, bytes);
            case 256032032: return cg_launch_cfg<256, 32, 8, 1, 32, 1>(P, epi, st, kid, bytes);
            default: return cg_launch_cfg<128, 128, 2, 2, 32, 1>(P, epi, st, kid, bytes);
        }
    }
    switch (key) {
        case 256256016: return cg_launch_cfg<256, 256, 2, 4, 16>(P, epi, st, kid, bytes);
        case 256256032: return cg_launch_cfg<256, 256, 2, 4, 32>(P, epi, st, kid, bytes);
        case 256128016: return cg_launch_cfg<256, 128, 4, 2, 16>(P, epi, st, kid, bytes);
        case 256032016: return cg_launch_cfg<256, 32, 8, 1, 16>(P, epi, st, kid, bytes);
        case 128128032: return cg_launch_cfg<128, 128, 2, 2, 32>(P, epi, st, kid, bytes);
        default: return cg_launch_cfg<128, 128, 2, 2, 16>(P, epi, st, kid, bytes);
    }
}

int64_t cg_fwd_row_bound(int Cin, int Cout, int k, int ops) { return ((int64_t)1 << (ops ? 30 : 31)) / std::max(Cout, k * Cin); }
int64_t cg_dgrad_row_bound(int Cin, int Cout, int k) { return ((int64_t)1 << 31) / std::max(Cin, k * Cout); }
int64_t cg_wgrad_grow_bound(int Cin, int Cout) { return ((int64_t)1 << 31) / std::max(Cout, Cin); }
int64_t cg_wgrad_xrow_bound(int Cin) { return ((int64_t)1 << 31) / Cin; }

}

VMASR_EXPORT void vmasr_conv_set_cu_limit(int32_t cus) { g_cg_cu_limit = cus < 0 ? 0 : cus; }
VMASR_EXPORT int32_t vmasr_conv_get_cu_limit(void) { return g_cg_cu_limit; }

VMASR_EXPORT int vmasr_conv_mfma_supported(int32_t Cin, int32_t Cout, int32_t k, int32_t stride) {
    const bool in_ok = Cin > 0 && (Cin % 128 == 0 || Cin == 32), out_ok = Cout > 0 && Cout % 128 == 0;
    return in_ok && out_ok && k >= 1 && k <= 8 && stride >= 1 && stride <= 3;
}

VMASR_EXPORT int vmasr_conv_mfma_supported_launch(int32_t Cin, int32_t Cout, int32_t k, int32_t stride, int32_t n, int64_t rows) {
    if (!vmasr_conv_mfma_supported(Cin, Cout, k, stride)) return 0;
    if (n < 1 || n > 8 || n * (stride + 1) > CG_MAXP) return 0;
    int64_t bound = std::min(cg_fwd_row_bound(Cin, Cout, k, 0), cg_dgrad_row_bound(Cin, Cout, k));
    bound = std::min(bound, std::min(cg_wgrad_grow_bound(Cin, Cout), cg_wgrad_xrow_bound(Cin)));
    if (Cin == 32) bound = std::min(bound, cg_fwd_row_bound(Cin, Cout, k, 1));
    return rows >= 1 && rows < bound ? 1 : 0;
}

VMASR_EXPORT int vmasr_conv_mfma_config(int32_t pass, int32_t Cin, int32_t Cout, int32_t ops, int32_t out[3]) {
    VMASR_REQUIRE(out && pass >= CG_PASS_FWD && pass <= CG_PASS_WGRAD && (ops == 0 || (ops == 1 && Cin == 32 && pass != CG_PASS_WGRAD)), VMASR_EINVAL,
                  "conv_mfma_config: pass 0..2, ops 0 or 1 (Cin 32, forward / input gradient), out");
    VMASR_REQUIRE(vmasr_conv_mfma_supported(Cin, Cout, 1, 1), VMASR_EINVAL, "conv_mfma_config: unsupported channel counts (Cin %d, Cout %d)", Cin, Cout);
    const CgConfig c = cg_config(pass, Cin, Cout, ops);
    out[0] = c.BM; out[1] = c.BN; out[2] = c.MF;
    return VMASR_OK;
}

namespace {
int cg_fwd(const vmasr_cg_slot *slots, int32_t n, int32_t Cin, int32_t Cout, int32_t k, int32_t stride, int32_t pad, int64_t rows_out,
           int32_t act, vmasr_stream_t stream, int ops) {
    const char *what = ops ? "conv_f32_fwd" : "conv_mfma_fwd";
    VMASR_REQUIRE(slots && n >= 1 && n <= CG_MAXP, VMASR_EINVAL, "%s: 1..%d slots", what, CG_MAXP);
    VMASR_REQUIRE(vmasr_conv_mfma_supported(Cin, Cout, k, stride) && (!ops || Cin == 32), VMASR_EINVAL,
                  "%s: unsupported shape (Cin %d, Cout %d, k %d, stride %d)", what, Cin, Cout, k, stride);
    VMASR_REQUIRE(rows_out % 256 == 0, VMASR_EINVAL, "%s: rows_out must be a multiple of 256", what);
    CgParams P = {};
    P.nprob = n;
    P.CA = Cin; P.NB = Cout; P.KB = k * Cin;
    double bytes = 0;
    for (int i = 0; i < n; ++i) {
        const vmasr_cg_slot &s = slots[i];
        VMASR_REQUIRE(s.ah && s.bh && s.c0 && (ops || (s.al && s.bl)), VMASR_EINVAL, "%s: null tensor in slot %d", what, i);
        VMASR_REQUIRE(!ops || (aligned_to(s.ah, 16) && aligned_to(s.bh, 16)), VMASR_EALIGN, "%s: slot %d: operands must be 16-byte aligned", what, i);
        const int64_t H1 = ((int64_t)s.H + 2 * pad - k) / stride + 1;
        const int64_t M = s.nseq * H1;
        VMASR_REQUIRE(H1 >= 1 && M <= rows_out && rows_out < cg_fwd_row_bound(Cin, Cout, k, ops), VMASR_EINVAL,
                      "%s: slot %d: %lld rows do not fit rows_out %lld (or 32-bit offsets)", what, i, (long long)M, (long long)rows_out);
        CgProb &p = P.prob[i];
        p.ah = (const bf16_t *)s.ah; p.al = (const bf16_t *)s.al; p.bh = (const bf16_t *)s.bh; p.bl = (const bf16_t *)s.bl;
        p.c0 = s.c0; p.c1 = s.c1; p.ch = (bf16_t *)s.ch; p.cl = (bf16_t *)s.cl; p.bias = s.bias;
        p.M = (int)M; p.Q = (int)H1; p.HA = s.H; p.HC = (int)H1;
        p.hq_mul = stride; p.hq_add = -pad; p.crow_mul = 1; p.crow_add = 0;
        p.ntaps = k; p.tap0 = 0; p.tap_step = 1; p.dstep = 1;
        p.zero_rows = (int)rows_out;
        bytes += (double)s.nseq * s.H * Cin * 4 + (double)Cout * k * Cin * 4 + (double)M * Cout * (act ? 12 : 4);
    }
    hipStream_t st = static_cast<hipStream_t>(stream);
    if (ops) VMASR_REQUIRE(Cout % 128 == 0, VMASR_EINVAL, "%s: Cout %% 128", what);
    return cg_launch(P, act != 0 ? 1 : 0, st, VMASR_K_CONV_MFMA_FWD, bytes, ops, true);
}
}

VMASR_EXPORT int vmasr_conv_mfma_fwd(const vmasr_cg_slot *slots, int32_t n, int32_t Cin, int32_t Cout, int32_t k, int32_t stride,
                                     int32_t pad, int64_t rows_out, int32_t act, vmasr_stream_t stream) {
    return cg_fwd(slots, n, Cin, Cout, k, stride, pad, rows_out, act, stream, 0);
}

VMASR_EXPORT int vmasr_conv_f32_fwd(const vmasr_cg_slot *slots, int32_t n, int32_t Cin, int32_t Cout, int32_t k, int32_t stride,
                                    int32_t pad, int64_t rows_out, int32_t act, vmasr_stream_t stream) {
    return cg_fwd(slots, n, Cin, Cout, k, stride, pad, rows_out, act, stream, 1);
}

namespace {

int cg_dgrad(const vmasr_cg_slot *slots, const vmasr_cg_gelu_bwd *epi, const float *gtok, int32_t n, int32_t Cin, int32_t Cout, int32_t k,
             int32_t stride, int32_t pad, int64_t rows_in, vmasr_stream_t stream, int ops = 0) {
    const char *what = ops ? "conv_f32_dgrad" : epi ? "conv_mfma_dgrad_gelu" : "conv_mfma_dgrad";
    VMASR_REQUIRE(!ops || (!epi && Cin == 32), VMASR_EINVAL, "%s: the f32 form serves Cin = 32 without a fused activation backward", what);
    VMASR_REQUIRE(slots && n >= 1 && n * (stride + 1) <= CG_MAXP, VMASR_EINVAL, "%s: too many slots", what);
    VMASR_REQUIRE(vmasr_conv_mfma_supported(Cin, Cout, k, stride), VMASR_EINVAL, "%s: unsupported shape (Cin %d, Cout %d, k %d, stride %d)", what,
                  Cin, Cout, k, stride);
    VMASR_REQUIRE(!epi || Cin % 128 == 0, VMASR_EINVAL, "%s: the fused activation backward needs Cin %% 128 == 0", what);
    CgParams P = {};
    P.CA = Cout; P.NB = Cin; P.KB = k * Cout;
    P.gtok = gtok;
    double bytes = 0;
    int np = 0;
    for (int i = 0; i < n; ++i) {
        const vmasr_cg_slot &s = slots[i];
        VMASR_REQUIRE(s.ah && s.bh && (ops || (s.al && s.bl)) && (epi ? (s.c0 || (s.ch && s.cl)) && (!s.ch == !s.cl) : s.c0 != nullptr), VMASR_EINVAL,
                      "%s: null tensor in slot %d", what, i);
        VMASR_REQUIRE(!ops || (aligned_to(s.ah, 16) && aligned_to(s.bh, 16)), VMASR_EALIGN, "%s: slot %d: operands must be 16-byte aligned", what, i);
        VMASR_REQUIRE(!epi || (epi[i].pre && epi[i].valid >= 0 && (!epi[i].sgn || gtok)), VMASR_EINVAL,
                      "%s: slot %d: pre-activation missing (or a sign map without the loss gradient)", what, i);
        const int64_t H = s.H, H1 = (H + 2 * pad - k) / stride + 1;
        VMASR_REQUIRE(H1 >= 1 && s.nseq * H <= rows_in && rows_in < cg_dgrad_row_bound(Cin, Cout, k), VMASR_EINVAL,
                      "%s: slot %d: %lld rows do not fit rows_in %lld (or 32-bit offsets)", what, i, (long long)(s.nseq * H), (long long)rows_in);
        auto outputs = [&](CgProb &p) {
            p.c0 = s.c0; p.c1 = nullptr; p.ch = nullptr; p.cl = nullptr; p.bias = nullptr;
            if (epi) {
                p.ch = (bf16_t *)s.ch; p.cl = (bf16_t *)s.cl;
                p.bias = epi[i].pre;
                p.c1 = reinterpret_cast<float *>(const_cast<signed char *>(epi[i].sgn));
                p.fscale = epi[i].scale;
                p.fvalid = (int)std::min<int64_t>(epi[i].valid, rows_in);
                p.db = epi[i].db;
            }
        };
        for (int r = 0; r < stride; ++r) {
            const int r0 = ((r - pad) % stride + stride) % stride;
            const int64_t Q = H > r0 ? (H - r0 + stride - 1) / stride : 0;
            if (Q == 0) continue;
            CgProb &p = P.prob[np++];
            p.ah = (const bf16_t *)s.ah; p.al = (const bf16_t *)s.al; p.bh = (const bf16_t *)s.bh; p.bl = (const bf16_t *)s.bl;
            outputs(p);
            p.M = (int)(s.nseq * Q); p.Q = (int)Q; p.HA = (int)H1; p.HC = (int)H;
            p.hq_mul = 1; p.hq_add = (r0 + pad - r) / stride;
            p.crow_mul = stride; p.crow_add = r0;
            p.ntaps = r < k ? (k - r + stride - 1) / stride : 0;
            p.tap0 = r; p.tap_step = stride; p.dstep = -1;
            p.zero_rows = 0;
        }
        if (s.nseq * H < rows_in) {
            CgProb &p = P.prob[np++];
            p.ah = (const bf16_t *)s.ah; p.al = (const bf16_t *)s.al; p.bh = (const bf16_t *)s.bh; p.bl = (const bf16_t *)s.bl;
            outputs(p);
            p.M = (int)(rows_in - s.nseq * H); p.Q = p.M; p.HA = 1; p.HC = 0;
            p.hq_mul = 0; p.hq_add = 0; p.crow_mul = 1; p.crow_add = (int)(s.nseq * H);
            p.ntaps = 0; p.tap0 = 0; p.tap_step = 1; p.dstep = 0;
            p.zero_rows = 0;
            p.db = nullptr;
        }
        bytes += (double)s.nseq * H1 * Cout * 4 + (double)Cout * k * Cin * 4 + (double)s.nseq * H * Cin * 4;
        if (epi) bytes += (double)s.nseq * H * Cin * ((s.c0 && s.ch ? 4.0 : 0.0) + 4.0 + (epi[i].sgn ? 1.0 : 0.0));
    }
    P.nprob = np;
    return cg_launch(P, epi ? 2 : 0, static_cast<hipStream_t>(stream), VMASR_K_CONV_MFMA_DGRAD, bytes, ops, false);
}

}

VMASR_EXPORT int vmasr_conv_mfma_dgrad(const vmasr_cg_slot *slots, int32_t n, int32_t Cin, int32_t Cout, int32_t k, int32_t stride,
                                       int32_t pad, int64_t rows_in, vmasr_stream_t stream) {
    return cg_dgrad(slots, nullptr, nullptr, n, Cin, Cout, k, stride, pad, rows_in, stream);
}

VMASR_EXPORT int vmasr_conv_f32_dgrad(const vmasr_cg_slot *slots, int32_t n, int32_t Cin, int32_t Cout, int32_t k, int32_t stride,
                                      int32_t pad, int64_t rows_in, vmasr_stream_t stream) {
// ... 54 lines not shown
```

### vm_asr_amd/discriminator.py

```python

import torch
import torch.nn as nn
import torch.nn.functional as F
from torch.nn.utils import parametrize
from torch.nn.utils.parametrizations import weight_norm

from . import _lib, knobs, mpd_ops as bind
from .linear import linear as _linear, weight_grad as _weight_grad
from .mpd_featloss import StackedFeatures, _FeatTapFn, _MaskedL1Fn, _masked_l1_ok, feature_loss_stacked
from .mpd_layers import (_BatchedLinearFn, _BatchedLinearSplitFn, _StackedConvFirstFn, _StackedConvMfmaFn, _StackedConvPostFn,
                         _StackedConvSplitFn, _StackedIm2ColFn, _UnstackRowsFn, _bmm3, _dw3, _l1_mode, _poison, _round_up, _split_k,
                         _split_mode, scores_only, skip_weight_grads)
from .mpd_link import _Link, _Tap
from .mpd_ops import SpectralBatch, _slot_arrays, geom_of as _geom, split_bf16

__all__ = ["PeriodDiscriminator", "MultiPeriodDiscriminator", "spectral_norm", "plain_torch_ops"]

_PLAIN_OPS = [False]


class plain_torch_ops:

    def __enter__(self):
        self._saved = _PLAIN_OPS[0]
        _PLAIN_OPS[0] = True
        return self

    def __exit__(self, *exc):
        _PLAIN_OPS[0] = self._saved
        return False


class _SpectralNorm(nn.Module):

    def __init__(self, weight, n_power_iterations=1, eps=1e-12):
        super().__init__()
        self.n_power_iterations, self.eps = n_power_iterations, eps
        w = weight.detach().flatten(1)
        u = F.normalize(w.new_empty(w.size(0)).normal_(0, 1), dim=0, eps=eps)
        v = F.normalize(w.new_empty(w.size(1)).normal_(0, 1), dim=0, eps=eps)
        self.register_buffer("_u", u)
        self.register_buffer("_v", v)
        self._power_method(w, 15)

    @torch.autograd.no_grad()
    def _power_method(self, w, n):
        if w.is_cuda and n > 0 and w.dtype == torch.float32:
            bind.spectral_power_iter(w.contiguous(), self._u, self._v, n, self.eps)
            return
        for _ in range(n):
            self._u = F.normalize((w @ self._v.unsqueeze(1)).squeeze(1), dim=0, eps=self.eps, out=self._u)
            self._v = F.normalize((w.t() @ self._u.unsqueeze(1)).squeeze(1), dim=0, eps=self.eps, out=self._v)

    def forward(self, weight):
        with torch.autocast(device_type=weight.device.type, enabled=False):
            pre = getattr(self, "_sigma_pre", None)
            if pre is not None and self.training and self.n_power_iterations == 0 and weight.dtype == torch.float32:
                return _SNDivFn.apply(weight, self._u, self._v, pre)
            w = (weight if weight.dtype == torch.float64 else weight.float()).flatten(1)
            if self.training:
                self._power_method(w, self.n_power_iterations)
            u, v = self._u.clone(), self._v.clone()
            sigma = (u * (w @ v.unsqueeze(1)).squeeze(1)).sum()
            return weight / sigma


class _SNDivFn(torch.autograd.Function):

    @staticmethod
    def forward(ctx, weight, u, v, sigma):
        out = weight / sigma
        ctx.save_for_backward(out, u, v, sigma)
        return out

    @staticmethod
    def backward(ctx, g):
        out, u, v, sigma = ctx.saved_tensors
        g2, o2 = g.reshape(u.numel(), -1), out.reshape(u.numel(), -1)
        s = torch.dot(g2.reshape(-1), o2.reshape(-1))
        gw = torch.addcmul(g2, (u * (-s)).unsqueeze(1), v.unsqueeze(0)) / sigma
        return gw.view_as(out), None, None, None


class _SNStackFn(torch.autograd.Function):

    @staticmethod
    def forward(ctx, n, *args):
        sig, us, vs, ws = args[:n], args[n:2 * n], args[2 * n:3 * n], args[3 * n:4 * n]
        pair_out = args[4 * n] if len(args) > 4 * n else None
        out = bind.sn_stack_fwd([w.detach().contiguous() for w in ws], sig, want_pair=pair_out is not None)
        if pair_out is not None:
            out, pair_out["w"] = out
# ... 160 lines not shown
    if x.is_cuda and ok and x.shape[2] + 2 * pad >= k:
        cdt = _lib.autocast_dtype(x)
        return _ConvKx1Fn.apply(x, weight, bias, stride, pad, cdt)
    return _conv_kx1_cl(x, weight, bias, stride, pad)


def _layer_path(li, act, cdt, prev_dt, stacked, k, stride, pad, Cin, Cout, n, rows_out, rows_in):
    f32 = cdt == torch.float32
    if (not act and prev_dt is not None and f32 and k == 3 and stride == 1 and pad == 1 and Cout == 1
            and prev_dt == torch.float32 and knobs.get("VMASR_CONV_POST") and bind.conv_post_supported(Cin, k)):
        return "post"
    if (act and li == 0 and f32 and k == 5 and stride == 3 and pad == 2 and Cout == 32 and k * Cin == 5 and Cin == 1
            and knobs.get("VMASR_CONV_FIRST")):
        return "first"
    if (f32 and knobs.get("VMASR_MPD_GEMM") == "bf16x3" and act and stacked
            and _batched_conv_mode() == "mfma"
            and (Cin >= 128 or _l1_mode() != "0")
            and bind.conv_mfma_supported_launch(Cin, Cout, k, stride, n, max(_round_up(rows_out, 256), rows_in))):
        return "mfma"
    if _split_mode(k * Cin, Cout, cdt) and Cin % 4 == 0:
        return "split"
    return "gemm"


class PeriodDiscriminator(nn.Module):
    def __init__(self, period, kernel_size=5, stride=3, use_spectral_norm=False, hidden=32):
        super().__init__()
        self.period = period
        norm = weight_norm if use_spectral_norm else spectral_norm
        pad = (kernel_size - 1) // 2
        chans = [1, hidden, hidden * 4, hidden * 16, hidden * 32]
        layers = [norm(nn.Conv2d(chans[i], chans[i + 1], (kernel_size, 1), (stride, 1), padding=(pad, 0)))
                  for i in range(4)]
        layers.append(norm(nn.Conv2d(hidden * 32, hidden * 32, (kernel_size, 1), 1, padding=(2, 0))))
        self.layers = nn.ModuleList(layers)
        self.conv_post = norm(nn.Conv2d(hidden * 32, 1, (3, 1), 1, padding=(1, 0)))

    def forward(self, x, detach_weights=False):
        fmap = []
        b, c, t = x.shape
        if t % self.period != 0:
            n_pad = self.period - (t % self.period)
            x = F.pad(x, (0, n_pad), "reflect")
            t = t + n_pad
        wb = (lambda l: (l.weight.detach(), l.bias.detach())) if detach_weights else (lambda l: (l.weight, l.bias))
        if not x.is_cuda or _PLAIN_OPS[0]:
            x = x.view(b, c, t // self.period, self.period)
            for layer in list(self.layers) + [self.conv_post]:
                w, bias = wb(layer)
                x = F.conv2d(x, w, bias, layer.stride, layer.padding)
                if layer is not self.conv_post:
                    x = F.gelu(x)
                fmap.append(x)
            return torch.flatten(x, 1, -1), fmap
        x = x.view(b, c, t // self.period, self.period).permute(0, 3, 2, 1)
        for layer in self.layers:
            w, bias = wb(layer)
            x = F.gelu(conv_kx1(x, w, bias, layer.stride[0], layer.padding[0]))
            fmap.append(x)
        w, bias = wb(self.conv_post)
        x = conv_kx1(x, w, bias, 1, self.conv_post.padding[0])
        fmap.append(x)
        return torch.flatten(x, 1, -1), fmap


class MultiPeriodDiscriminator(nn.Module):
    def __init__(self, hidden=32, periods=(2, 3, 5, 7, 11)):
        super().__init__()
        self.discriminators = nn.ModuleList([PeriodDiscriminator(p, hidden=hidden) for p in periods])
        self._frozen = None

    def frozen_weights(self):
        import contextlib

        @contextlib.contextmanager
        def ctx():
            object.__setattr__(self, "_frozen", {})
            try:
                yield
            finally:
                object.__setattr__(self, "_frozen", None)
        return ctx()

    def _forward_batched(self, x, detach_weights=False):
        discs = list(self.discriminators)
        n, (B, _, T) = len(discs), x.shape
        cdt = _lib.autocast_dtype(x)
        cur = []
        for d in discs:
            xp, p = x, d.period
            if T % p:
                xp = F.pad(xp, (0, p - T % p), "reflect")
            cur.append(xp.view(B, 1, -1, p).permute(0, 3, 2, 1).to(cdt))
        fmaps, stacks, valid, taps = [[] for _ in discs], [], [], []
        next_pair = this_link = None
        for li in range(len(discs[0].layers) + 1):
            layers = [d.layers[li] if li < len(d.layers) else d.conv_post for d in discs]
            k, stride, pad = layers[0].kernel_size[0], layers[0].stride[0], layers[0].padding[0]
            P = [c.shape[1] for c in cur]
            H1 = [(c.shape[2] + 2 * pad - k) // stride + 1 for c in cur]
            Ms = [B * p * h for p, h in zip(P, H1)]
            act = li < len(discs[0].layers)
            sgeom, src = None, cur
            pair, next_pair = next_pair, None
            prev_link, this_link = this_link, None
            if stacks and stacks[-1].dtype == cdt and knobs.get("VMASR_STACK_INPUT"):
                sgeom, src = tuple((B * p, c.shape[2]) for c, p in zip(cur, P)), (stacks[-1],)
            rows = _round_up(max(Ms), 256)
            Cin = cur[0].shape[3]
            path = _layer_path(li, act, cdt, stacks[-1].dtype if stacks else None, sgeom is not None, k, stride, pad, Cin,
                               layers[0].out_channels, n, max(Ms), max(B * p * c.shape[2] for c, p in zip(cur, P)))
            wcache = wpair = None
            if path == "mfma" and self._frozen is not None:
                wcache = self._frozen.setdefault(("mfma_ops", li), {})
            W = None
            if knobs.get("VMASR_SN_STACK"):
                key = (li, bool(detach_weights))
                W = self._frozen.get(key) if self._frozen is not None else None
                if W is None:
                    got = {} if (path == "mfma" and not (Cin < 128 and _l1_mode() == "f32")
                                 and (wcache is None or "ops" not in wcache)) else None
                    W = _sn_stack(layers, got)
                    wpair = got.get("w") if got is not None else None
                    if W is not None and detach_weights:
                        W = W.detach()
                    if W is not None and self._frozen is not None:
                        self._frozen[key] = W
            if W is not None:
                ws = [(None, l.bias.detach() if detach_weights else l.bias) for l in layers]
            else:
                ws = [(l.weight.detach(), l.bias.detach()) if detach_weights else (l.weight, l.bias) for l in layers]
                W = torch.stack([w.squeeze(3).transpose(1, 2) for w, _ in ws])
                W = W.reshape(n, W.shape[1], -1)
            bstack = torch.stack([b for _, b in ws])
            if path == "post":
                y = _StackedConvPostFn.apply(tuple(valid[-1]), tuple(c.shape[2] for c in cur), W, bstack, stacks[-1], prev_link)
            elif path == "first":
                y = _StackedConvFirstFn.apply(rows, W, bstack, *cur)
            elif path == "mfma":
                xh, xl = pair if pair is not None else (None, None)
                this_link = _Link()
                y = _StackedConvMfmaFn.apply(k, stride, pad, rows, sgeom, wcache, W, bstack, src[0], xh, xl, this_link, prev_link, wpair)
                next_pair, this_link.pair = this_link.pair, None
            elif path == "split":
                y = _StackedConvSplitFn.apply(k, stride, pad, rows, act, sgeom, W, bstack, *src)
            else:
                cols = _StackedIm2ColFn.apply(k, stride, pad, rows, sgeom, *src)
                y = _BatchedLinearFn.apply(cols, W, bstack, cdt, act)
            tap = None
            if (act and y.requires_grad and y.dtype == torch.float32 and x.requires_grad
                    and knobs.get("VMASR_FEAT_TAP")):
                t = _Tap()
                y, token = _FeatTapFn.apply(y, t)
                tap = (token, t)
                if this_link is not None:
                    this_link.tap = t
            outs = _UnstackRowsFn.apply(y, *Ms)
            cur = [o.view(B, p, h, -1) for o, p, h in zip(outs, P, H1)]
            for f, c in zip(fmaps, cur):
                f.append(c)
            stacks.append(y)
            valid.append(tuple(Ms))
            taps.append(tap)
        return [torch.flatten(c, 1, -1) for c in cur], StackedFeatures(fmaps, stacks, valid, taps)

    def _use_batched(self, x):
        return (x.is_cuda and not _PLAIN_OPS[0] and knobs.get("VMASR_MPD_BATCHED")
                and len(self.discriminators) > 1)

    def forward_single(self, x, detach_weights=False):
        if self._use_batched(x):
            return self._forward_batched(x, detach_weights)
        res = [d(x, detach_weights) for d in self.discriminators]
        return [r[0] for r in res], [r[1] for r in res]

    def forward_pair(self, y, y_hat):
        n = y.shape[0]
        y_real, y_gen, fmap_real, fmap_gen = [], [], [], []
        both = torch.cat((y, y_hat), dim=0)
        if self._use_batched(both):
            scores, feats = self._forward_batched(both)
            y_real, y_gen = [s[:n] for s in scores], [s[n:] for s in scores]
            fmap_real = StackedFeatures([[t[:n] for t in f] for f in feats], feats.stacks, [tuple(m // 2 for m in v) for v in feats.valid])
            return y_real, y_gen, fmap_real, [[t[n:] for t in f] for f in feats]
        else:
            res = [d(both) for d in self.discriminators]
        for s, f in res:
            y_real.append(s[:n]); y_gen.append(s[n:])
            fmap_real.append([t[:n] for t in f]); fmap_gen.append([t[n:] for t in f])
        return y_real, y_gen, fmap_real, fmap_gen

    def spectral_norms(self):
        return [m for m in self.modules() if isinstance(m, _SpectralNorm)]

    def power_iterate_all(self, n_iter, with_sigma=False):
        pairs = [(mod.parametrizations.weight[0], mod.parametrizations.weight.original)
                 for mod in self.modules() if isinstance(mod, nn.Conv2d) and parametrize.is_parametrized(mod, "weight")
                 and isinstance(mod.parametrizations.weight[0], _SpectralNorm)]
        if not pairs or not all(w.is_cuda and w.dtype == torch.float32 for _, w in pairs) or len(pairs) > 64:
            return False
        weights = [w.detach() for _, w in pairs]
        batch = getattr(self, "_sn_batch", None)
        if batch is None or not batch.matches(weights):
            batch = SpectralBatch([m for m, _ in pairs], weights)
            object.__setattr__(self, "_sn_batch", batch)
        batch.run(n_iter, with_sigma)
        return True

    def clear_sigmas(self):
        batch = getattr(self, "_sn_batch", None)
        if batch is not None:
            batch.clear_sigma()

    def forward(self, y, y_hat):
        y_real, y_gen, fmap_real, fmap_gen = [], [], [], []
        for disc in self.discriminators:
            r, fr = disc(y)
            y_real.append(r)
            fmap_real.append(fr)
            if y_hat is not None:
                g, fg = disc(y_hat)
                y_gen.append(g)
                fmap_gen.append(fg)
            else:
                y_gen.append(0)
                fmap_gen.append(0)
        return y_real, y_gen, fmap_real, fmap_gen
```

### vm_asr_amd/knobs.py

```python
import os
import warnings
from collections import namedtuple

Knob = namedtuple("Knob", "name kind default values reader doc parse")


def _bad(k, raw, allowed):
    return ValueError(f"{k.name}={raw!r}: expected {allowed}")


def _flag(k, raw):
    if raw == "1":
        return True
    if raw == "0":
        return False
    raise _bad(k, raw, "0 or 1")


def _choice(k, raw):
    if raw in k.values:
        return raw
    raise _bad(k, raw, "one of " + " | ".join(k.values))


# ... 10 lines not shown
    except ValueError:
        raise _bad(k, raw, "a number") from None


def _str(k, raw):
    return raw or k.default


def _comma_list(k, raw):
    return tuple(raw.split(","))


def _step_variant(k, raw):
    if raw == "":
        return None
    if raw == "one":
        return (False, None)
    if raw == "lane":
        return (True, None)
    if raw.startswith("lane:"):
        try:
            share = float(raw[5:])
        except ValueError:
            share = 0.0
        if 0.0 < share < 1.0:
            return (True, share)
    raise _bad(k, raw, "one | lane | lane:<share> with 0 < share < 1")


_PARSE = {"flag": _flag, "choice": _choice, "int": _int, "float": _float, "str": _str}
_FLAG_VALUES = ("0", "1")


def _k(name, kind, default, doc, values=None, reader="python", parse=None):
    if kind == "flag":
        values, default = _FLAG_VALUES, bool(default)
    return Knob(name, kind, default, values, reader, doc, parse or _PARSE.get(kind))


def _csrc(name, default, doc):
    return Knob(name, "csrc", default, None, "csrc", doc, None)


def _external(name, doc):
    return Knob(name, "external", None, None, "external", doc, None)


KNOBS = {k.name: k for k in (
    _k("VMASR_LIB", "str", None, "path of the HIP library instead of vm_asr_amd/libvmasr_hip.so (A/B and sanitizer builds); read at import"),
    _k("VMASR_DETERMINISTIC", "flag", 0, "ordered fp32 accumulation everywhere; every stream-layout decision then keeps one stream (_lib.det_mode())"),
    _k("VMASR_LINEAR_F64ACC", "choice", "auto", "fp32 Linear with float64 accumulation: 1 always, 0 never, auto only where no gradient is recorded",
       values=("auto", "0", "1")),
    _k("VMASR_SKINNY", "choice", "1", "streaming kernel for Linear layers of many rows and few features: 1 where it beats the GEMM library, 0 off, "
       "all every supported shape", values=("1", "0", "all")),
    _k("VMASR_SPLITK_CHUNK", "int", 2048, "fewest rows of one K-split of a weight-gradient GEMM; read at import"),
    _k("VMASR_XPROJ_MAX_D", "int", 512, "largest d_inner that takes the x_proj row kernels instead of einsums; read at import"),
    _k("VMASR_FUSED_MLP", "flag", 1, "LayerNorm + Mlp + residual of a VSS block as one operator (mlp.py)"),
    _k("VMASR_FUSED_INPROJ", "flag", 1, "LayerNorm + in_proj + split + SiLU as one operator (inproj.py)"),
    _k("VMASR_FUSED_OUTPROJ", "flag", 1, "out_proj + DropPath + residual as one operator (outproj.py)"),
    _k("VMASR_SS2D_FUSED", "flag", 1, "the d_state-1 SS2D core (x_proj, dt_proj, four-direction scan, merge) as one operator (ss2d_core.py)"),
    _k("VMASR_SS2D_DEEP", "flag", 1, "the deep stages' SS2D core on the row-parallel kernels (ss2d_deep.py)"),
    _k("VMASR_SS2D_GLUE", "flag", 1, "the pre-scan and gated-LayerNorm glue kernels (ss2d_glue.py)"),
    _k("VMASR_SS2D_PAIRS", "flag", 1, "magnitude and phase blocks of equal shape through one gated-LayerNorm launch (ss2d_glue.py)"),
    _k("VMASR_IM2COL2D", "flag", 1, "the generator's 2-D convolutions through the row-major im2col kernel (model.py)"),
    _k("VMASR_STFT_LOSS", "flag", 1, "the multi-resolution STFT loss kernel (loss.py)"),
    _k("VMASR_LSGAN", "flag", 1, "the least-squares GAN loss kernel (loss.py)"),
    _k("VMASR_MPD_BATCHED", "flag", 1, "all period discriminators layer by layer on stacked operands"),
    _k("VMASR_MPD_GEMM", "choice", "bf16x3", "fp32 discriminator GEMMs as bf16x3 MFMA triples, or fp32 library GEMMs", values=("bf16x3", "fp32")),
    _k("VMASR_MPD_CONV", "choice", None, "ONE variable read at two sites.  conv_kx1 (one discriminator at a time; unset = unfold): gemm = the "
       "im2col-free GEMM form for stride 3 and stride 1, s3 = that form for the stride-3 layers only, unfold or mfma = unfold + GEMM.  "
       "Batched path (unset = mfma): mfma = the implicit-GEMM MFMA kernels for the compute-bound layers, gemm / s3 / unfold = not those",
       values=("mfma", "gemm", "s3", "unfold")),
    _k("VMASR_MPD_CONV_L1", "choice", "f32", "the 32 -> 128 layer: f32 exact-fp32 MFMA implicit GEMM, 1 bf16x3 pairs, 0 library GEMMs",
       values=("f32", "1", "0")),
    _k("VMASR_MPD_SPLIT_MIN", "int", 1 << 18, "smallest K * N of a stacked layer that takes the split (hi, lo) GEMM path"),
    _k("VMASR_MPD_KCAT", "flag", 0, "the split GEMM's three products as one GEMM over a concatenated K"),
    _k("VMASR_MPD_FUSE_GELU_BWD", "flag", 1, "the activation backward inside the input-gradient epilogue"),
    _k("VMASR_SN_STACK", "flag", 1, "spectral normalisation, stack and permutation of a layer's weights in one launch"),
    _k("VMASR_STACK_INPUT", "flag", 1, "a layer reads the previous layer's stacked output directly"),
    _k("VMASR_CONV_POST", "flag", 1, "the 1-channel output convolution straight on the stacked maps"),
    _k("VMASR_CONV_FIRST", "flag", 1, "the 1 -> 32 channel input convolution + GELU straight from the folded signals"),
    _k("VMASR_FEAT_TAP", "flag", 1, "a feature map's gradient (next layer's + feature-matching loss's) formed in one pass"),
    _k("VMASR_FEAT_L1", "flag", 1, "the feature-matching loss on the stacked maps in one kernel"),
    _k("VMASR_MSD_CONV", "choice", "hip", "the MSD's strided grouped 1-D convolutions: hip = the exact-fp32 MFMA kernels (csrc/gconv1d.hip), "
       "torch = F.conv1d (A/B measurements, double backward)", values=("hip", "torch"), reader="python:msd"),
    _k("VMASR_MSD_STEM", "choice", "hip", "the MSD's 1 -> hidden stem convolution + GELU: hip = one fused pass that keeps no pre-activation "
       "(csrc/stem1d.hip), torch = F.conv1d + F.gelu (A/B measurements, double backward)", values=("hip", "torch"), reader="python:msd"),
    _k("VMASR_MSD_FEAT", "choice", "hip", "the MSD's feature-matching loss in the generator's pass: hip = formed on the way (the stem's share inside "
       "the stem kernels, the other maps in the one-pass L1 kernel; msd_featmatch.py), torch = forward_single + the loop of sub, abs, mean",
       values=("hip", "torch"), reader="python:msd"),
    _k("VMASR_MSD_TAIL", "choice", "torch", "the MSD's dense tail (8h -> 8h k 5 + GELU, conv_post): hip = the exact-fp32 MFMA kernels with ordered "
       "split-K sums (csrc/dconv1d.hip: bit-identical run to run, no library algorithm search), torch = F.conv1d + F.gelu (the default: "
       "faster on the 8h -> 8h layer, profiles/msd_tail.md; double backward)", values=("hip", "torch"), reader="python:msd"),
    _k("VMASR_TWO_STREAM", "choice", "1", "the discriminator on a side stream: 1 on, 0 one stream, force also in deterministic mode (test hook)",
       values=("1", "0", "force")),
    _k("VMASR_SHARE_FAKE_PASS", "flag", 1, "one discriminator pass over the fake batch serves both phases of the step"),
    _k("VMASR_GEN_STREAMS", "choice", "auto", "the generator's phase branch on a stream of its own in captured steps: auto where the trainer says so, "
       "1 off, 2 on, 2eager on in eager steps too (debugging aid)", values=("auto", "1", "2", "2eager")),
    _k("VMASR_GEN_LANES", "list", None, "comma list of the segments that leave the main stream (pe,e0..e3,d0..d3,out,ia); unset = all (dev aid)",
       parse=_comma_list),
    _k("VMASR_STEP_VARIANT", "variant", None, "pins the captured step layout: one | lane | lane:<share of the CUs for the discriminator's backward>",
       values=("one", "lane", "lane:0.75"), parse=_step_variant),
    _k("VMASR_SIDE_CUS", "int", None, "CU limit of the discriminator's convolutions beside the generator's backward (and forward unless "
       "VMASR_SIDE_CUS_FWD is set); 0 = no limit; unset = Trainer.side_cu_limits()"),
    _k("VMASR_SIDE_CUS_FWD", "int", None, "the same beside the generator's forward"),
    _k("VMASR_SIDE_CUS_MINC", "int", 0, "the backward limit only for layers at least this wide"),
    _k("VMASR_GRAPH_GC_GUARD", "flag", 1, "no cyclic garbage collection between a graph capture and its first replays"),
    _k("VMASR_PHASE_EVENTS", "flag", 0, "device-clock marks at the step's phase boundaries (tools/phase_probe.py)"),
    _k("VMASR_LN_DEFER", "flag", 1, "LayerNorm's dgamma / dbeta of a whole backward pass reduced in one launch"),
    _k("VMASR_HIP_ADAMW", "flag", 1, "the multi-tensor AdamW kernel on the flat gradient buffers"),
    _k("VMASR_FUSED_ADAMW", "flag", 1, "torch's fused AdamW where the HIP kernel does not apply"),
    _k("VMASR_LP_SHADOWS", "flag", 1, "bf16 shadow copies of the parameters, refreshed by the optimiser kernel"),
    _k("VMASR_LP_SHADOWS_T", "flag", 1, "transposed bf16 shadows of the 2-D weights too"),
    _k("VMASR_RESUME_CONFIG_MISMATCH", "choice", "raise", "a checkpoint written under another configuration: raise or warn", values=("raise", "warn")),
    _k("VMASR_DIST_BACKEND", "str", None, "torch.distributed backend; unset = nccl on a GPU, else gloo"),
    _k("VMASR_DIST_TIMEOUT_S", "int", 600, "process-group timeout in seconds"),
    _k("VMASR_RCCL_TIMEOUT_S", "float", 300.0, "watchdog of a captured collective in seconds (rccl.py)"),
    _k("VMASR_RCCL_DIRECT", "flag", 0, "the trainer's own RCCL communicator outside captures too"),
    _k("VMASR_GRAPH_COLLECTIVES", "flag", 0, "capture the gradient all-reduces into the step's graph"),
    _k("VMASR_OVERLAP_REDUCE", "flag", 1, "asynchronous gradient all-reduces; 0 = strictly between the graphs"),
    _k("VMASR_GRAD_COMM", "choice", "fp32", "wire dtype of the gradient all-reduce: fp32, mpd-bf16 the discriminator's as bf16, bf16 both",
       values=("fp32", "mpd-bf16", "bf16")),
    _k("VMASR_GRAD_COMM_EMULATE", "choice", None, "one rank: the 16-bit wire's rounding applied to this rank's own gradient", values=("mpd-bf16", "bf16")),
    _csrc("VMASR_CONV_CU_SLACK", 24, "convgemm.hip: CUs by which the convolution CU limit is soft"),
    _csrc("VMASR_CONV_TILE", 0, "convgemm.hip: 128 forces the small tile"),
    _csrc("VMASR_CONV_MFMA", 16, "convgemm.hip: 16 = the 16x16x32 MFMA form, 32 = 32x32x16"),
    _csrc("VMASR_CONV_F32_TILE", 128, "convgemm.hip: tile of the exact-fp32 form, 128 or 256"),
    _csrc("VMASR_XPROJ_MFMA", 0, "xproj.hip: 1 = the MFMA kernels (measured slower)"),
    _csrc("VMASR_SSCAN_N_RB", 0, "sscan_n.hip: rows per workgroup; 0 = planned"),
    _csrc("VMASR_SSCAN_N_PP", 0, "sscan_n.hip: state pairs per wave; 0 = planned"),
    _csrc("VMASR_BWD_WAVES", 0, "sscan.hip: waves of the d_state-1 backward; 0 = 8"),
    _csrc("VMASR_SSCAN_N_LEGACY", 0, "sscan.hip: non-zero = the one-state-at-a-time kernels for general d_state (A/B)"),
    _external("VMASR_BENCH_WATCHDOG", "bench.py: seconds after which a wedged run dumps its stacks and exits"),
    _external("VMASR_PARITY_TABLE", "tests/conftest.py: path of the achieved-error table the session writes"),
    _external("VMASR_TEST_CLIPS", "tests/test_fullsize.py: clips of the full-size accuracy test"),
    _external("VMASR_ORACLE_LIB", "oracle/oracle.py: path of the oracle library (sanitizer build)"),
    _external("VMASR_REFERENCE", "tests/golden/_refload.py: checkout of the reference project that regenerates the goldens"),
)}


def get(name):
    k = KNOBS[name]
    raw = os.environ.get(name)
    return k.default if raw is None else k.parse(k, raw)


def undeclared():
    return sorted(n for n in os.environ if n.startswith("VMASR_") and n not in KNOBS)


def warn_undeclared():
    names = undeclared()
    if names:
        warnings.warn(f"unknown VMASR_* variables in the environment (ignored): {', '.join(names)}; vm_asr_amd/knobs.py lists the switches",
                      stacklevel=2)
```

### vm_asr_amd/mpd_featloss.py

```python
import torch

from . import knobs, mpd_ops as bind


class StackedFeatures(list):

    def __init__(self, per_disc, stacks, valid, taps=None):
        super().__init__(per_disc)
        self.stacks, self.valid = stacks, valid
        self.taps = taps if taps is not None else [None] * len(stacks)

    def detach(self):
        return StackedFeatures([[f.detach() for f in fs] for fs in self], [y.detach() for y in self.stacks], self.valid)


class _FeatTapFn(torch.autograd.Function):

    @staticmethod
    def forward(ctx, y, tap):
        ctx.tap = tap
        ctx.set_materialize_grads(False)
        return y.view_as(y), y.new_zeros(1)

    @staticmethod
    def backward(ctx, gy, gtok):
        t = ctx.tap
        sgn = t.sgn
        t.gtok = None
        consumed, t.consumed = t.consumed, False
        if consumed:
            return gy, None
        if gtok is None or sgn is None:
            return gy, None
        add = None if gy is None else gy.float().contiguous()
        return bind.masked_l1_bwd(sgn, gtok.float().contiguous(), t.valid, t.scale, add, tap=True), None


_FEAT_MASKS = {}


class _MaskedL1Fn(torch.autograd.Function):

    @staticmethod
    def forward(ctx, real, gen, valid, scale, token, tap):
        tapped = token is not None and ctx.needs_input_grad[4]
        partials, sgn = bind.masked_l1_fwd(real, gen, valid, scale, ctx.needs_input_grad[1] or tapped)
        ctx.meta = (valid, scale, gen.shape)
        ctx.tapped = tapped
        ctx.tap = tap if tapped else None
        if tapped:
            tap.offer(sgn, valid, scale)
        elif sgn is not None:
            ctx.save_for_backward(sgn)
        return partials.sum().float()

    @staticmethod
    def backward(ctx, g):
        if ctx.tapped:
            ctx.tap.gtok = g.detach().reshape(1).float().contiguous()
            return None, None, None, None, g.reshape(1), None
        (sgn,) = ctx.saved_tensors
        valid, scale, _ = ctx.meta
        return None, bind.masked_l1_bwd(sgn, g.float().contiguous(), valid, scale), None, None, None, None


def _masked_l1_ok(yr, yg):
    return (yg.is_cuda and yr.is_cuda and yg.dtype == torch.float32 and yr.dtype == torch.float32 and yg.is_contiguous()
            and yr.is_contiguous() and not yr.requires_grad and yg.shape[0] <= 8 and yg.shape[0] == yr.shape[0]
            and (yg.shape[1] * yg.shape[2]) % 4 == 0 and (yr.shape[1] * yr.shape[2]) % 4 == 0
            and knobs.get("VMASR_FEAT_L1"))


def feature_loss_stacked(real, gen):
    if not (isinstance(real, StackedFeatures) and isinstance(gen, StackedFeatures)) or real.valid != gen.valid:
        return None
    n_maps = sum(len(fs) for fs in gen)
    total = None
    for yr, yg, valid, tap in zip(real.stacks, gen.stacks, real.valid, gen.taps):
        R, N = min(yr.shape[1], yg.shape[1]), yg.shape[2]
        if max(valid) > R:
            return None
        if _masked_l1_ok(yr, yg):
            scale = tuple(1.0 / (m * N * n_maps) for m in valid)
            if tap is not None and tap[0].requires_grad and not tap[1].fed:
                term = _MaskedL1Fn.apply(yr, yg.detach(), tuple(valid), scale, *tap)
            else:
                term = _MaskedL1Fn.apply(yr, yg, tuple(valid), scale, None, None)
            total = term if total is None else total + term
            continue
        key = (yg.device, valid, R, N, n_maps)
        mask = _FEAT_MASKS.get(key)
        if mask is None:
            rows = torch.arange(R, device=yg.device).unsqueeze(0)
            m = torch.tensor(valid, device=yg.device).unsqueeze(1)
            mask = ((rows < m).float() / (m.float() * N * n_maps)).unsqueeze(2)
            _FEAT_MASKS[key] = mask
        term = ((yg[:, :R] - yr[:, :R]).abs() * mask).sum()
        total = term if total is None else total + term
    return total
```

### vm_asr_amd/mpd_layers.py

```python
import torch
import torch.nn.functional as F

from . import _lib, knobs, mpd_ops as bind
from .linear import _mm_acc
from .mpd_ops import geom_of as _geom, split_bf16



def _round_up(v, m):
    return -(-v // m) * m


class _StackedIm2ColFn(torch.autograd.Function):

    @staticmethod
    def forward(ctx, k, stride, pad, rows, geom, *xs):
        if geom is not None:
            src = xs[0].contiguous()
            ctx.geom = (k, stride, pad, None, tuple(geom), tuple(src.shape))
        else:
            src, geom = [x.contiguous() for x in xs], _geom(xs)
            ctx.geom = (k, stride, pad, [tuple(x.shape) for x in xs], None, None)
        return bind.im2col_kx1(src, geom, src[0].shape[-1], k, stride, pad, rows)

# ... 174 lines not shown
        kcat = fused and knobs.get("VMASR_MPD_KCAT")
        if kcat:
            acat = bind.im2col_kx1_split(src, geom, C, k, stride, pad, rows, cat3=True)
            ch, cl = acat[:, :, :K], acat[:, :, K:2 * K]
        else:
            ch, cl = bind.im2col_kx1_split(src, geom, C, k, stride, pad, rows)
        wcat = bind.weight_prep_split(w)
        wth, wtl = wcat[:, :, :N], wcat[:, :, 2 * N:]
        b32 = bias.detach().float().contiguous()
        pre = None
        if kcat:
            f32 = torch.float32
            wk = torch.cat((wth, wth, wtl), dim=1)
            pre = torch.bmm(acat, wk, out_dtype=f32)
            y = bind.bias_gelu_fwd(pre, b32)
        elif fused:
            f32 = torch.float32
            parts = torch.empty((3, n, rows, N), dtype=f32, device=dev)
            torch.bmm(ch, wth, out_dtype=f32, out=parts[0])
            torch.bmm(cl, wth, out_dtype=f32, out=parts[1])
            torch.bmm(ch, wtl, out_dtype=f32, out=parts[2])
            pre = parts[0]
            y = bind.bias_gelu_fwd(parts, b32, 3)
        else:
            y = _bmm3(ch, cl, wth, wtl)
            y.add_(b32.unsqueeze(1))
            if act:
                pre = y
                y = F.gelu(pre)
        ctx.save_for_backward(ch, cl, wcat, *([pre] if pre is not None else []))
        ctx.geom = (k, stride, pad, [tuple(x.shape) for x in xs], weight.dtype, bias.dtype, [x.dtype for x in xs], act, fused, sgeom)
        return y

    @staticmethod
    def backward(ctx, gy):
        ch, cl, wcat, *rest = ctx.saved_tensors
        k, stride, pad, shapes, wdt, bdt, xdts, act, fused, sgeom = ctx.geom
        gy = gy.float().contiguous()
        n, M, N = gy.shape
        K = ch.shape[2]
        want_db = ctx.needs_input_grad[7] and not skip_weight_grads.on
        want_dx = any(ctx.needs_input_grad[8:])
        db32 = gcat = None
        if N % 4 == 0 and N <= 1024:
            db32, = _lib.zeros_f32(gy.device, (n, N) if want_db else None)
            gh, gl, gcat = bind.gelu_bwd_split(rest[0] if act else None, gy, db32, cat=want_dx)
        else:
            if act:
                gy = torch.ops.aten.gelu_backward(gy, rest[0])
            gh, gl = split_bf16(gy)
            db32 = gy.sum(1) if want_db else None
        dxs = [None] * len(shapes)
        if want_dx:
            if gcat is None:
                gcat = torch.cat((gh, gl, gh), dim=2)
            dcols = torch.bmm(gcat, wcat.transpose(1, 2), out_dtype=torch.float32)
            if sgeom is not None:
                dxs = [bind.col2im_kx1_stacked(dcols, sgeom, shapes[0], k, stride, pad).to(xdts[0])]
            else:
                outs = bind.col2im_kx1_multi(dcols, shapes, k, stride, pad, ctx.needs_input_grad[8:])
                dxs = [o.to(xdts[i]) if o is not None else None for i, o in enumerate(outs)]
        dw = db = None
        if not skip_weight_grads.on:
            if ctx.needs_input_grad[6]:
                dw = _dw3(gh, gl, ch, cl, wdt)
            if ctx.needs_input_grad[7]:
                db = db32.to(bdt)
        return (None, None, None, None, None, None, dw, db, *dxs)


def _dgrad_operand(ops, key, pair, w, k, n, N, C):
    if key not in ops:
        if bind.weight_transpose_supported(N, C):
            ops[key] = bind.weight_transpose(w, k, pair=pair)
        else:
            wt = w.view(n, N, k, C).permute(0, 3, 2, 1).reshape(n, C, k * N).contiguous()
            ops[key] = split_bf16(wt) if pair else wt
    return ops[key]


class _StackedConvMfmaFn(torch.autograd.Function):

    @staticmethod
    def forward(ctx, k, stride, pad, rows, geom, wcache, weight, bias, x, xh, xl, link, below=None, wpair=None):
        from . import convgemm as cg
        x_req = x.requires_grad
        x = x.float().contiguous()
        w = weight.detach().float().contiguous()
        f32 = x.shape[2] < 128 and _l1_mode() == "f32"
        ops = wcache.get("ops") if wcache is not None else None
        if ops is None:
            ops = {} if f32 else {"w": wpair if wpair is not None else split_bf16(w)}
            if wcache is not None:
                wcache["ops"] = ops
        if f32:
            pre, y, yh, yl = cg.conv_fwd_f32(x, w, bias.detach().float().contiguous(), geom, k, stride, pad, rows, act=True)
            xh = xl = x
        else:
            if xh is None:
                xh, xl = split_bf16(x)
            wh, wl = ops["w"]
            pre, y, yh, yl = cg.conv_fwd(xh, xl, wh, wl, bias.detach().float().contiguous(), geom, k, stride, pad, rows, act=True)
        ctx.save_for_backward(xh, xl, pre, w)
        ctx.f32 = f32
        ctx.meta = (k, stride, pad, tuple(geom), ops, weight.dtype, bias.dtype, x.shape)
        ctx.link, ctx.below = link, below
        link.fill(pre, x.shape[2], x_req, weight.requires_grad, bias.requires_grad, pair=(yh, yl))
        return y

    @staticmethod
    def _fuse_below(ctx, gh, gl, wth, wtl, geom, k, stride, pad, rows_in, skip_w):
        from . import convgemm as cg
        plan = ctx.below.plan(skip_w, scores_only.on) if ctx.below is not None else None
        if plan is None:
            return False
        db32 = _lib.zeros_f32(gh.device, (gh.shape[0], wth.shape[1]))[0] if plan.want_db else None
        g32, pair = cg.conv_dgrad_gelu(gh, gl, wth, wtl, geom, k, stride, pad, rows_in, ctx.below.pre, want_f32=plan.want_f32,
                                       want_pair=plan.want_pair, db=db32, **(plan.loss or {}))
        ctx.below.put(g32, pair, db32)
        return True

    @staticmethod
    def backward(ctx, gy):
        from . import convgemm as cg
        xh, xl, pre, w = ctx.saved_tensors
        k, stride, pad, geom, ops, wdt, bdt, xshape = ctx.meta
        n, M, N = gy.shape
        C = xshape[2]
        skip_w = skip_weight_grads.on
        want_db = ctx.needs_input_grad[7] and not skip_w
        fp32_dgrad = C < 128 and ctx.needs_input_grad[8]
        need_pair = (not fp32_dgrad and ctx.needs_input_grad[8]) or (ctx.needs_input_grad[6] and not skip_w)
        gh = gl = gx = None
        stash = ctx.link.take()
        if stash is not None:
            gx, pair_, db32 = stash
            gh, gl = pair_ if pair_ is not None else (None, None)
            if (want_db and db32 is None) or (need_pair and gh is None) or (fp32_dgrad and gx is None):
                raise RuntimeError("MPD: the fused activation backward left less than this layer's backward needs")
        if stash is None:
            gy = gy.float().contiguous()
            db32, = _lib.zeros_f32(gy.device, (n, N) if want_db else None)
            if need_pair:
                gh, gl, _ = bind.gelu_bwd_split(pre, gy, db32)
            if fp32_dgrad:
                gx, _ = bind.gelu_bwd(pre, gy, None if need_pair else db32)
        dx = dw = db = None
        if fp32_dgrad and ctx.f32:
            dx = cg.conv_dgrad_f32(gx, _dgrad_operand(ops, "wt32", False, w, k, n, N, C), geom, k, stride, pad, xshape[1])
        elif fp32_dgrad:
            dx = bind.col2im_kx1_stacked(torch.bmm(gx, w), geom, xshape, k, stride, pad)
        elif ctx.needs_input_grad[8]:
            wth, wtl = _dgrad_operand(ops, "wt", True, w, k, n, N, C)
            if _StackedConvMfmaFn._fuse_below(ctx, gh, gl, wth, wtl, geom, k, stride, pad, xshape[1], skip_w):
                dx = _poison(gy.device).expand(xshape)
            else:
                dx = cg.conv_dgrad(gh, gl, wth, wtl, geom, k, stride, pad, xshape[1])
        if not skip_w:
            if ctx.needs_input_grad[6]:
                if ctx.f32:
                    xh, xl = split_bf16(xh)
                dw = cg.conv_wgrad(gh, gl, xh, xl, geom, k, stride, pad).to(wdt)
            if want_db:
                db = db32.to(bdt)
        return (None, None, None, None, None, None, dw, db, dx, None, None, None, None, None)


_POISON = {}


def _poison(device):
    t = _POISON.get(device)
    if t is None:
        t = _POISON[device] = torch.full((), float("nan"), dtype=torch.float32, device=device)
    return t


def _l1_mode():
    return knobs.get("VMASR_MPD_CONV_L1")


class _StackedConvFirstFn(torch.autograd.Function):

    @staticmethod
    def forward(ctx, rows, W, bias, *xs):
        xcs = [x.float().contiguous() for x in xs]
        w32, b32 = W.detach().float().contiguous(), bias.detach().float().contiguous()
        pre, act = bind.conv_first_fwd(xcs, _geom(xcs), w32, b32, rows)
        ctx.save_for_backward(pre, w32, *xcs)
        ctx.meta = (W.dtype, bias.dtype, [x.dtype for x in xs], [tuple(x.shape) for x in xs])
        return act

    @staticmethod
    def backward(ctx, gy):
        pre, w32, *xcs = ctx.saved_tensors
        wdt, bdt, xdts, shapes = ctx.meta
        gy = gy.float().contiguous()
        skip_w = skip_weight_grads.on
        want_dw, want_db = ctx.needs_input_grad[1] and not skip_w, ctx.needs_input_grad[2] and not skip_w
        want_dx = any(ctx.needs_input_grad[3:])
        dxs = [None] * len(xcs)
        dcols, dw, db = bind.conv_first_bwd(xcs, _geom(shapes), w32, pre, gy, want_dx, want_dw, want_db)
        if want_dx:
            outs = bind.col2im_kx1_multi(dcols, shapes, 5, 3, 2, ctx.needs_input_grad[3:])
            dxs = [o.to(xdts[i]) if o is not None else None for i, o in enumerate(outs)]
        return (None, dw.to(wdt) if want_dw else None, db.to(bdt) if want_db else None, *dxs)


class _StackedConvPostFn(torch.autograd.Function):

    @staticmethod
    def forward(ctx, Ms, Hs, W, bias, x, below=None):
        xc, w32, b32 = x.contiguous(), W.detach().float().contiguous(), bias.detach().float().contiguous()
        y = bind.conv_post_fwd(xc, w32, b32, Ms, Hs)
        ctx.save_for_backward(xc, w32)
        ctx.meta = (tuple(Ms), tuple(Hs), W.dtype, bias.dtype, tuple(bias.shape))
        ctx.below = below
        return y

    @staticmethod
    def _fuse_below(ctx, xc, w32, gy, Ms, Hs, want_dw, want_db, skip_w):
        plan = ctx.below.plan(skip_w, scores_only.on, map_shape=xc.shape) if ctx.below is not None else None
        if plan is None:
            return None
        g32, pair, dbcol, dw, db = bind.conv_post_bwd_gelu(xc, w32, gy, ctx.below.pre, Ms, Hs, plan.want_pair, plan.want_f32, want_dw, want_db,
                                                           plan.want_db, **(plan.loss or {}))
        ctx.below.put(g32, pair, dbcol)
        return dw, db

    @staticmethod
    def backward(ctx, gy):
        xc, w32 = ctx.saved_tensors
        Ms, Hs, wdt, bdt, bshape = ctx.meta
        gy = gy.float().contiguous()
        skip_w = skip_weight_grads.on
        want_dx, want_dw, want_db = ctx.needs_input_grad[4], ctx.needs_input_grad[2] and not skip_w, ctx.needs_input_grad[3] and not skip_w
        fused = _StackedConvPostFn._fuse_below(ctx, xc, w32, gy, Ms, Hs, want_dw, want_db, skip_w) if want_dx else None
        if fused is not None:
            (dw, db), dx = fused, _poison(gy.device).expand(xc.shape)
        else:
            dx, dw, db = bind.conv_post_bwd(xc, w32, gy, Ms, Hs, want_dx, want_dw, want_db)
        return (None, None, dw.to(wdt) if want_dw else None, db.view(bshape).to(bdt) if want_db else None, dx, None)


class _UnstackRowsFn(torch.autograd.Function):

    @staticmethod
    def forward(ctx, y, *Ms):
# ... 19 lines not shown
```

### vm_asr_amd/trainer.py

```python
import math
import os
import time

import torch
import torch.distributed as dist
from torch.nn.parallel import DistributedDataParallel as DDP

from . import knobs
from . import metric as metric_mod
from .data import SyntheticVCTK
from .grad_sync import FlatGrads
from .loss import HiFiGANLoss, MultiResolutionSTFTLoss, mae_loss, mse_loss
from .optim import (_RUNTIME_GROUP_KEYS, CosineWarmupScheduler, build_optimizer, load_optimizer_state, lr_to_device,
                    portable_optimizer_state, set_weight_decay, unwrap)

__all__ = ["BaseTrainer", "Trainer", "SyntheticVCTK", "CosineWarmupScheduler", "build_optimizer",
           "set_weight_decay", "init_distributed", "unwrap"]


def init_distributed():
    world = int(os.environ.get("WORLD_SIZE", "1"))
    rank = int(os.environ.get("RANK", "0"))
    local = int(os.environ.get("LOCAL_RANK", "0"))
    if world > 1 and not dist.is_initialized():
# ... 380 lines not shown

    def _two_streams(self):
        from . import _lib, hip_env
        mode = knobs.get("VMASR_TWO_STREAM")
        if mode not in ("1", "force") or (_lib.det_mode() and mode != "force"):
            return False
        if not self._share_fake_pass():
            return False
        if not hip_env.streamk_dp_in_force():
            if not self._warned_streamk:
                self._warned_streamk = True
                import warnings
                warnings.warn("TENSILE_STREAMK_DATA_PARALLEL=1 is not known to be in force: the train step stays on one HIP stream "
                              "(vm_asr_amd/hip_env.py sets it when the package is imported before the GPU is initialised)")
            return False
        return True

    def side_cu_limits(self, lanes=False):
        cus = torch.cuda.get_device_properties(self.device).multi_processor_count
        dims = self.config.MODEL.VSSM.DIMS
        dims = dims[0] if isinstance(dims, (list, tuple)) else dims
        r8 = lambda v: max(8, int(round(v / 8.0)) * 8)
        batch = self._step_batch or self.config.DATA.BATCH_SIZE
        bwd = 1 / 2 if dims >= 32 else (3 / 4 if lanes and batch <= 4 else 5 / 8)
        share = self._lane_bwd_share
        if lanes and share is not None:
            bwd = share
        return r8(cus * 3 / 8), r8(cus * bwd)

    def _side_cus(self, forward=False):
        from . import convgemm
        lanes = (self.device.type == "cuda" and torch.cuda.is_current_stream_capturing()
                 and bool(getattr(unwrap(self.models["generator"]), "phase_lane", False)))
        fwd_auto, bwd_auto = self.side_cu_limits(lanes)
        cus = knobs.get("VMASR_SIDE_CUS_FWD") if forward else None
        if cus is None:
            cus = knobs.get("VMASR_SIDE_CUS")
        if cus is None:
            cus = fwd_auto if forward else bwd_auto
        return convgemm.cu_limit(cus, 0 if forward else knobs.get("VMASR_SIDE_CUS_MINC"))

    def _mark(self, name, stream=None):
        if not knobs.get("VMASR_PHASE_EVENTS"):
            return
        from . import _lib
        if self._phase_buf is None:
            self._phase_buf = torch.zeros(64, dtype=torch.int64, device=self.device)
        slot = self.phase_marks.setdefault(name, len(self.phase_marks))
        st = stream if stream is not None else torch.cuda.current_stream(self.device)
        _lib.check(_lib.lib().vmasr_mark_time(self._phase_buf.data_ptr() + 8 * slot, st.cuda_stream), "mark_time")

    def _side_stream(self):
        if self._side is None:
            self._side = torch.cuda.Stream(self.device)
        return self._side

    def _forward_losses(self, wave_input, wave_target, highcut):
        acc = self._acc
        self._set_deferred_reductions()
        shared = self._share_fake_pass()
        two = shared and self._two_streams()
        dev_t = self.device.type
        step_amp = lambda: torch.autocast(device_type=dev_t, dtype=torch.bfloat16, enabled=self.amp and self.amp_scope == "step")
        d_losses = {}
        if two:
            import contextlib
            main, side = torch.cuda.current_stream(self.device), self._side_stream()
            mpd = unwrap(self.models["mpd"])
            with contextlib.ExitStack() as weights:
                self._mark("start", main)
                side.wait_stream(main)
                with torch.cuda.stream(side), step_amp(), self._side_cus(forward=True):
                    weights.enter_context(self._mpd_weights_once())
                    y_real, f_real = mpd.forward_single(wave_target)
                    self._mark("d_real_fwd_end", side)
                with torch.autocast(device_type=dev_t, dtype=torch.bfloat16, enabled=self.amp):
                    wave_out = self.models["generator"](wave_input, highcut)
                wave_f = wave_out.float()
                self._mark("g_fwd_end", main)
                wave_d = wave_f.detach().requires_grad_(True)
                side.wait_stream(main)
                wave_d.record_stream(side)
                with torch.cuda.stream(side), step_amp():
                    y_fake, f_fake = mpd.forward_single(wave_d)
                    d_losses = {"mpd": self.higi_gan_loss.discriminator_loss(y_real, y_fake)}
                    f_real = _detach_fmaps(f_real)
                    g_side = self._generator_losses(wave_d, wave_target, f_real, fake_pass=(y_fake, f_fake), parts=("mpd",))
                    total_d = sum(d_losses.values()) / acc
                    g_mpd = sum(g_side.values()) / acc if g_side else None
                    self._mark("d_fake_fwd_losses_end", side)
                with step_amp():
                    g_losses = self._generator_losses(wave_f, wave_target, parts=("signal",))
                    g_sig = sum(g_losses.values()) / acc if g_losses else None
            main.wait_stream(side)
            for v in list(g_side.values()) + [total_d]:
                v.record_stream(main)
            g_losses.update(g_side)
            two = {"wave_f": wave_f, "wave_d": wave_d, "g_sig": g_sig, "g_mpd": g_mpd}
        else:
            with torch.autocast(device_type=dev_t, dtype=torch.bfloat16, enabled=self.amp):
                wave_out = self.models["generator"](wave_input, highcut)
            with step_amp():
                with self._mpd_weights_once():
                    if shared:
                        mpd = unwrap(self.models["mpd"])
                        y_real, f_real = mpd.forward_single(wave_target)
                        y_fake, f_fake = mpd.forward_single(wave_out.float())
                        d_losses = {"mpd": self.higi_gan_loss.discriminator_loss(y_real, y_fake)}
                        f_real = _detach_fmaps(f_real)
                        g_losses = self._generator_losses(wave_out, wave_target, f_real, fake_pass=(y_fake, f_fake))
                    else:
                        d_losses, fmap_real = self._discriminator_losses(wave_out, wave_target)
                        g_losses = self._generator_losses(wave_out, wave_target, fmap_real)
            total_d = sum(d_losses.values()) / acc if self.gan else None
        with torch.set_grad_enabled(not two):
            total_g = sum(g_losses.values()) / acc
        logs = {"total_loss": total_g.detach()}
        logs.update({f"generator/{k}": v.detach() for k, v in g_losses.items()})
        if self.gan:
            logs["total_disc_loss"] = total_d.detach()
        return {"wave_out": wave_out, "total_g": total_g, "total_d": total_d, "shared": shared, "two": two, "logs": logs}

    def _backward_d(self, st, zero=True):
        if not self.gan:
            return
        keys = self._d_keys()
        if zero:
            for key in keys:
                self.grads.zero(key, self.optimizer_D)
        if st["shared"]:
            st["total_d"].backward(inputs=self.grads.targets("mpd"), retain_graph=True)
        else:
            st["total_d"].backward()
        for key in keys:
            self.grads.gather(key)

    def _backward_g(self, st, zero=True):
        from . import layernorm
        try:
            if zero:
                self.grads.zero("generator", self.optimizer_G)
            if st["shared"]:
                from .discriminator import skip_weight_grads
                with skip_weight_grads():
                    st["total_g"].backward(inputs=self.grads.targets("generator"))
            else:
                st["total_g"].backward()
        finally:
            layernorm.DEFER_REDUCE = False
            layernorm.reset_uses()
        self.grads.gather("generator")

    def _backward_two(self, st, zero=True, reduce=False):
        from . import layernorm
        from .discriminator import scores_only, skip_weight_grads
        tw = st["two"]
        main, side = torch.cuda.current_stream(self.device), self._side_stream()
        try:
            with torch.cuda.stream(side):
                if tw["g_mpd"] is not None:
                    with skip_weight_grads():
                        tw["g_mpd"].backward(inputs=[tw["wave_d"]], retain_graph=True)
                handed = torch.cuda.Event()
                handed.record(side)
                self._mark("g_dgrad_end", side)
                side.wait_stream(main)
                if zero:
                    self.grads.zero("mpd", self.optimizer_D)
                with self._side_cus(), scores_only():
                    st["total_d"].backward(inputs=self.grads.targets("mpd"))
                self.grads.gather("mpd")
                self._mark("d_bwd_end", side)
                if reduce and self.gan:
                    self.grads.reduce("mpd", async_op=True)
            main.wait_event(handed)
            if zero:
                self.grads.zero("generator", self.optimizer_G)
            roots, seeds = [], []
            if tw["g_sig"] is not None:
                roots.append(tw["g_sig"])
                seeds.append(None)
            gw = tw["wave_d"].grad
            if gw is not None:
                gw.record_stream(main)
                roots.append(tw["wave_f"])
                seeds.append(gw)
            torch.autograd.backward(roots, seeds, inputs=self.grads.targets("generator"))
        finally:
            layernorm.DEFER_REDUCE = False
            layernorm.reset_uses()
        self.grads.gather("generator")
        self._mark("g_bwd_end", main)
# ... 393 lines not shown
```

Baseline: 198.9 clips/s.

## Fuse MPD feature-matching L1 into fake-pass conv forward epilogue

Adds a conv forward epilogue that takes the bf16-pair MPD layers of the fake pass, computes the GELU output, compares it with the real pass' feature map, and writes per-tile L1 partial sums and sign maps. The fake pass then skips the separate L1 kernel and the fp32 feature maps that only the loss reads. This cuts memory traffic and kernel launches. In exchange it adds a double-precision reduction and extra reads of the real map inside the epilogue, and it reorders detach so the real maps are available before the fake forward.

```diff
diff --git a/include/vmasr_hip.h b/include/vmasr_hip.h
--- a/include/vmasr_hip.h
+++ b/include/vmasr_hip.h
@@ -225,6 +225,16 @@
 } vmasr_cg_gelu_bwd;
 int vmasr_conv_mfma_dgrad_gelu(const vmasr_cg_slot *slots, const vmasr_cg_gelu_bwd *epi, const float *gtok, int32_t n, int32_t Cin, int32_t Cout,
                                int32_t k, int32_t stride, int32_t pad, int64_t rows_in, vmasr_stream_t stream);
+typedef struct vmasr_cg_match {
+    const float *real;
+    void *sgn;
+    int64_t valid;
+    float scale;
+    int32_t reserved;
+} vmasr_cg_match;
+int vmasr_conv_mfma_fwd_match(const vmasr_cg_slot *slots, const vmasr_cg_match *match, double *partials, int32_t n, int32_t Cin, int32_t Cout,
+                              int32_t k, int32_t stride, int32_t pad, int64_t rows_out, vmasr_stream_t stream);
+int64_t vmasr_conv_mfma_fwd_match_partials(int32_t n, int32_t Cin, int32_t Cout, int64_t rows_out);
 
 int vmasr_wgrad_finish_multi(const float *const *parts, float *const *dws, float *const *dbs, float *const *e1s, float *const *e2s,
                              const int32_t *Ss, const int32_t *Ns, const int32_t *Ks, const int32_t *lds, int32_t n, vmasr_stream_t stream);
@@ -488,6 +498,7 @@
     VMASR_K_DCONV1D_REDUCE,
     VMASR_K_DCONV1D_WGRAD,
     VMASR_K_DCONV1D_WGRAD_REDUCE,
+    VMASR_K_CONV_MFMA_FWD_MATCH,
     VMASR_K_RESAMPLE,
     VMASR_K_COUNT
 };
diff --git a/vm_asr_amd/_lib.py b/vm_asr_amd/_lib.py
--- a/vm_asr_amd/_lib.py
+++ b/vm_asr_amd/_lib.py
@@ -49,6 +49,10 @@
 
 class CgGeluBwd(ctypes.Structure):
     _fields_ = [("pre", c_vp), ("sgn", c_vp), ("valid", c_i64), ("scale", ctypes.c_float), ("reserved", c_i32), ("db", c_vp)]
+
+
+class CgMatch(ctypes.Structure):
+    _fields_ = [("real", c_vp), ("sgn", c_vp), ("valid", c_i64), ("scale", ctypes.c_float), ("reserved", c_i32)]
 
 
 class SS2DDeepParams(ctypes.Structure):
@@ -143,6 +147,9 @@
     "vmasr_conv_set_cu_limit": (None, [c_i32]),
     "vmasr_conv_get_cu_limit": (c_i32, []),
     "vmasr_conv_mfma_fwd": (ctypes.c_int, [ctypes.POINTER(CgSlot), c_i32, c_i32, c_i32, c_i32, c_i32, c_i32, c_i64, c_i32, c_vp]),
+    "vmasr_conv_mfma_fwd_match": (ctypes.c_int, [ctypes.POINTER(CgSlot), ctypes.POINTER(CgMatch), c_vp, c_i32, c_i32, c_i32, c_i32, c_i32, c_i32, c_i64,
+                                                 c_vp]),
+    "vmasr_conv_mfma_fwd_match_partials": (c_i64, [c_i32, c_i32, c_i32, c_i64]),
     "vmasr_conv_mfma_dgrad": (ctypes.c_int, [ctypes.POINTER(CgSlot), c_i32, c_i32, c_i32, c_i32, c_i32, c_i32, c_i64, c_vp]),
     "vmasr_conv_f32_fwd": (ctypes.c_int, [ctypes.POINTER(CgSlot), c_i32, c_i32, c_i32, c_i32, c_i32, c_i32, c_i64, c_i32, c_vp]),
     "vmasr_conv_f32_dgrad": (ctypes.c_int, [ctypes.POINTER(CgSlot), c_i32, c_i32, c_i32, c_i32, c_i32, c_i32, c_i64, c_vp]),
@@ -331,7 +338,7 @@
     return t2 if t2.is_contiguous() else t2.contiguous()
 
 
-K_COUNT = 78
+K_COUNT = 79
 
 
 def zeros_f32(device, *shapes):
diff --git a/vm_asr_amd/convgemm.py b/vm_asr_amd/convgemm.py
--- a/vm_asr_amd/convgemm.py
+++ b/vm_asr_amd/convgemm.py
@@ -85,6 +85,36 @@
     return _fwd(_lib.lib().vmasr_conv_mfma_fwd, xh, xl, wh, wl, bias, geom, k, stride, pad, rows_out, act, want_pair)
 
 
+def match_partials(n, Cin, Cout, rows_out):
+    return int(_lib.lib().vmasr_conv_mfma_fwd_match_partials(int(n), int(Cin), int(Cout), int(rows_out)))
+
+
+def conv_fwd_match(xh, xl, wh, wl, bias, geom, k, stride, pad, rows_out, real, valid, scale, partials=None, want_y=False):
+    _need(xh, xl, wh, wl, bias, real, partials)
+    (n, _, Cin), Cout, dev = xh.shape, wh.shape[1], xh.device
+    npart = match_partials(n, Cin, Cout, rows_out)
+    if npart < 0:
+        raise RuntimeError(f"conv_fwd_match: no matching epilogue for {n} slots of {Cin} -> {Cout} channels")
+    assert real.shape == (n, rows_out, Cout) and real.dtype == torch.float32 and len(valid) == len(scale) == n
+    if partials is None:
+        partials = torch.empty(npart, dtype=torch.float64, device=dev)
+    assert partials.shape == (npart,) and partials.dtype == torch.float64
+    pre = torch.empty((n, rows_out, Cout), dtype=torch.float32, device=dev)
+    y = torch.empty_like(pre) if want_y else None
+    yh = torch.empty((n, rows_out, Cout), dtype=torch.bfloat16, device=dev)
+    yl = torch.empty_like(yh)
+    sgn = torch.empty((n, rows_out, Cout), dtype=torch.int8, device=dev)
+    sl = _slots(geom, ah=xh, al=xl, bh=wh, bl=wl, c0=pre, c1=y, ch=yh, cl=yl, bias=bias)
+    mt = (_lib.CgMatch * n)()
+    for i in range(n):
+        mt[i].real = _ptr(real, i, rows_out * Cout * 4)
+        mt[i].sgn = _ptr(sgn, i, rows_out * Cout)
+        mt[i].valid, mt[i].scale = int(valid[i]), float(scale[i])
+    _apply_limit(Cin, Cout)
+    _lib.call(_lib.lib().vmasr_conv_mfma_fwd_match, sl, mt, partials, n, Cin, Cout, k, stride, pad, rows_out, device=dev)
+    return pre, y, yh, yl, sgn, partials
+
+
 def conv_dgrad(gh, gl, wth, wtl, geom, k, stride, pad, rows_in):
     return _dgrad(_lib.lib().vmasr_conv_mfma_dgrad, gh, gl, wth, wtl, geom, k, stride, pad, rows_in)
 
diff --git a/vm_asr_amd/csrc/api.hip b/vm_asr_amd/csrc/api.hip
--- a/vm_asr_amd/csrc/api.hip
+++ b/vm_asr_amd/csrc/api.hip
@@ -40,7 +40,8 @@
     "conv_mfma_fwd", "conv_mfma_dgrad", "conv_mfma_wgrad", "wgrad_finish", "skinny_linear", "metrics", "resample_design", "degrade_batch",
     "gconv1d_fwd", "gconv1d_dgrad", "gconv1d_wgrad", "gconv1d_wgrad_reduce",
     "stem1d_fwd", "stem1d_bwd", "stem1d_bwd_reduce",
-    "dconv1d_fwd", "dconv1d_dgrad", "dconv1d_reduce", "dconv1d_wgrad", "dconv1d_wgrad_reduce", "resample_poly"};
+    "dconv1d_fwd", "dconv1d_dgrad", "dconv1d_reduce", "dconv1d_wgrad", "dconv1d_wgrad_reduce",
+    "conv_mfma_fwd_match", "resample_poly"};
 }
 
 bool g_prof_on = false;
diff --git a/vm_asr_amd/csrc/convgemm.hip b/vm_asr_amd/csrc/convgemm.hip
--- a/vm_asr_amd/csrc/convgemm.hip
+++ b/vm_asr_amd/csrc/convgemm.hip
@@ -18,6 +18,7 @@
 constexpr int CG_BM = 128, CG_BN = 128, CG_BK = 32;
 constexpr int CG_TILE = CG_BM * CG_BK * 2;
 constexpr int CG_STAGE = 4 * CG_TILE;
+constexpr int CG_MATCH_SLOTS = 8;
 constexpr int CG_MAXP = 24;
 
 struct CgProb {
@@ -45,6 +46,9 @@
     int NB;
     int KB;
     const float *gtok;
+    const float *mreal[CG_MATCH_SLOTS];
+    signed char *msgn[CG_MATCH_SLOTS];
+    double *partials;
 };
 static_assert(sizeof(CgParams) <= 4096, "CgParams is passed by value as the kernel's argument block");
 
@@ -55,6 +59,8 @@
 __device__ __forceinline__ float cg_gelu_grad(float x) {
     return 0.5f * (1.f + erff(x * 0.70710678118654752f)) + x * 0.3989422804014327f * __expf(-0.5f * x * x);
 }
+
+__device__ __forceinline__ signed char cg_sgn1(float d) { return (signed char)((d > 0.f) - (d < 0.f)); }
 
 __device__ __forceinline__ f32x16 cg_mfma(const bf16x8 a, const bf16x8 b, const f32x16 c) {
     return __builtin_amdgcn_mfma_f32_32x32x16_bf16(a, b, c, 0, 0, 0);
@@ -255,6 +261,7 @@
     float4 bias4 = make_float4(0.f, 0.f, 0.f, 0.f);
     float4 dbs = make_float4(0.f, 0.f, 0.f, 0.f);
     float gs = 0.f;
+    double macc = 0.0;
     if constexpr (EPI == 2) {
         if (pr.c1 && P.gtok) gs = P.gtok[0] * pr.fscale;
     } else {
@@ -312,6 +319,32 @@
                 }
                 continue;
             }
+            if constexpr (EPI == 3) {
+                *reinterpret_cast<float4 *>(pr.c0 + o) = v;
+                float yy[4] = {0.f, 0.f, 0.f, 0.f};
+                if (live) { yy[0] = cg_gelu(v.x); yy[1] = cg_gelu(v.y); yy[2] = cg_gelu(v.z); yy[3] = cg_gelu(v.w); }
+#pragma unroll
+                for (int e = 0; e < 4; ++e) asm volatile("" : "+v"(yy[e]));
+                if (pr.c1) *reinterpret_cast<float4 *>(pr.c1 + o) = make_float4(yy[0], yy[1], yy[2], yy[3]);
+                union { uint2 raw; bf16_t e[4]; } hh, ll;
+#pragma unroll
+                for (int e = 0; e < 4; ++e) {
+                    hh.e[e] = (bf16_t)yy[e];
+                    ll.e[e] = (bf16_t)(yy[e] - (float)hh.e[e]);
+                }
+                *reinterpret_cast<uint2 *>(pr.ch + o) = hh.raw;
+                *reinterpret_cast<uint2 *>(pr.cl + o) = ll.raw;
+                char4 q;
+                q.x = q.y = q.z = q.w = 0;
+                if (live && cr < pr.fvalid) {
+                    const float4 b = *reinterpret_cast<const float4 *>(P.mreal[pi] + o);
+                    const float d0 = yy[0] - b.x, d1 = yy[1] - b.y, d2 = yy[2] - b.z, d3 = yy[3] - b.w;
+                    macc += (double)((fabsf(d0) + fabsf(d1)) + (fabsf(d2) + fabsf(d3)));
+                    q.x = cg_sgn1(d0); q.y = cg_sgn1(d1); q.z = cg_sgn1(d2); q.w = cg_sgn1(d3);
+                }
+                *reinterpret_cast<char4 *>(P.msgn[pi] + o) = q;
+                continue;
+            }
             *reinterpret_cast<float4 *>(pr.c0 + o) = v;
             if constexpr (ACT) {
                 float4 y = make_float4(0.f, 0.f, 0.f, 0.f);
@@ -342,6 +375,19 @@
                 for (int q = 0; q < RPI; ++q) t += ct[q * BN + tid];
                 atomicAdd(pr.db + n0 + tid, t);
             }
+        }
+    }
+    if constexpr (EPI == 3) {
+        for (int off = 32; off > 0; off >>= 1) macc += __shfl_down(macc, off, 64);
+        __syncthreads();
+        double *wsum = reinterpret_cast<double *>(smem);
+        if (lane == 0) wsum[wave] = macc;
+        __syncthreads();
+        if (tid == 0) {
+            double tot = 0.0;
+#pragma unroll
+            for (int w = 0; w < NT / 64; ++w) tot += wsum[w];
+            P.partials[t] = tot * (double)pr.fscale;
         }
     }
     __syncthreads();
@@ -592,6 +638,8 @@
         (void)hipFuncSetAttribute(reinterpret_cast<const void *>(&conv_mfma_nt_kernel<BM, BN, WM, WN, 0, MF, OPS>), hipFuncAttributeMaxDynamicSharedMemorySize, (int)smem);
         if constexpr (HAS_EPI2)
             (void)hipFuncSetAttribute(reinterpret_cast<const void *>(&conv_mfma_nt_kernel<BM, BN, WM, WN, 2, MF, OPS>), hipFuncAttributeMaxDynamicSharedMemorySize, (int)smem);
+        if constexpr (HAS_EPI2)
+            (void)hipFuncSetAttribute(reinterpret_cast<const void *>(&conv_mfma_nt_kernel<BM, BN, WM, WN, 3, MF, OPS>), hipFuncAttributeMaxDynamicSharedMemorySize, (int)smem);
         attr_done = true;
     }
     if (epi == 1) {
@@ -603,6 +651,13 @@
             set_error("conv_mfma: no fused activation backward for this tile");
             return VMASR_EINVAL;
         }
+    } else if (epi == 3) {
+        if constexpr (HAS_EPI2) {
+            VMASR_LAUNCH(kid, bytes, (conv_mfma_nt_kernel<BM, BN, WM, WN, 3, MF, OPS>), dim3(cg_grid(tiles, smem)), dim3(64 * WM * WN), smem, st, P);
+        } else {
+            set_error("conv_mfma: no matching forward epilogue for this tile");
+            return VMASR_EINVAL;
+        }
     } else {
         VMASR_LAUNCH(kid, bytes, (conv_mfma_nt_kernel<BM, BN, WM, WN, 0, MF, OPS>), dim3(cg_grid(tiles, smem)), dim3(64 * WM * WN), smem, st, P);
     }
@@ -703,8 +758,13 @@
 
 namespace {
 int cg_fwd(const vmasr_cg_slot *slots, int32_t n, int32_t Cin, int32_t Cout, int32_t k, int32_t stride, int32_t pad, int64_t rows_out,
-           int32_t act, vmasr_stream_t stream, int ops) {
-    const char *what = ops ? "conv_f32_fwd" : "conv_mfma_fwd";
+           int32_t act, vmasr_stream_t stream, int ops, const vmasr_cg_match *match = nullptr, double *partials = nullptr) {
+    const char *what = match ? "conv_mfma_fwd_match" : ops ? "conv_f32_fwd" : "conv_mfma_fwd";
+    if (match) {
+        VMASR_REQUIRE(!ops && partials && aligned_to(partials, 8) && n >= 1 && n <= CG_MATCH_SLOTS, VMASR_EINVAL,
+                      "%s: bf16-pair form, a partials buffer and 1..%d slots", what, CG_MATCH_SLOTS);
+        VMASR_REQUIRE(Cin % 128 == 0, VMASR_EINVAL, "%s: offered on the 128- and 256-wide tiles only (Cin %% 128 == 0)", what);
+    }
     VMASR_REQUIRE(slots && n >= 1 && n <= CG_MAXP, VMASR_EINVAL, "%s: 1..%d slots", what, CG_MAXP);
     VMASR_REQUIRE(vmasr_conv_mfma_supported(Cin, Cout, k, stride) && (!ops || Cin == 32), VMASR_EINVAL,
                   "%s: unsupported shape (Cin %d, Cout %d, k %d, stride %d)", what, Cin, Cout, k, stride);
@@ -728,10 +788,26 @@
         p.hq_mul = stride; p.hq_add = -pad; p.crow_mul = 1; p.crow_add = 0;
         p.ntaps = k; p.tap0 = 0; p.tap_step = 1; p.dstep = 1;
         p.zero_rows = (int)rows_out;
-        bytes += (double)s.nseq * s.H * Cin * 4 + (double)Cout * k * Cin * 4 + (double)M * Cout * (act ? 12 : 4);
+        bytes += (double)s.nseq * s.H * Cin * 4 + (double)Cout * k * Cin * 4;
+        if (match) {
+            const vmasr_cg_match &mt = match[i];
+            VMASR_REQUIRE(s.ch && s.cl && mt.real && mt.sgn && mt.valid >= 0 && aligned_to(mt.real, 16) && aligned_to(mt.sgn, 4), VMASR_EINVAL,
+                          "%s: slot %d: the bf16 pair, the real map (16-byte aligned) and the sign map (4-byte aligned) are required", what, i);
+            P.mreal[i] = mt.real;
+            P.msgn[i] = static_cast<signed char *>(mt.sgn);
+            p.fscale = mt.scale;
+            p.fvalid = (int)std::min<int64_t>(mt.valid, rows_out);
+            bytes += (double)M * Cout * (s.c1 ? 12 : 8) + (double)std::min<int64_t>(p.fvalid, M) * Cout * 5;
+        } else {
+            bytes += (double)M * Cout * (act ? 12 : 4);
+        }
     }
     hipStream_t st = static_cast<hipStream_t>(stream);
     if (ops) VMASR_REQUIRE(Cout % 128 == 0, VMASR_EINVAL, "%s: Cout %% 128", what);
+    if (match) {
+        P.partials = partials;
+        return cg_launch(P, 3, st, VMASR_K_CONV_MFMA_FWD_MATCH, bytes, 0, true);
+    }
     return cg_launch(P, act != 0 ? 1 : 0, st, VMASR_K_CONV_MFMA_FWD, bytes, ops, true);
 }
 }
@@ -739,6 +815,18 @@
 VMASR_EXPORT int vmasr_conv_mfma_fwd(const vmasr_cg_slot *slots, int32_t n, int32_t Cin, int32_t Cout, int32_t k, int32_t stride,
                                      int32_t pad, int64_t rows_out, int32_t act, vmasr_stream_t stream) {
     return cg_fwd(slots, n, Cin, Cout, k, stride, pad, rows_out, act, stream, 0);
+}
+
+VMASR_EXPORT int vmasr_conv_mfma_fwd_match(const vmasr_cg_slot *slots, const vmasr_cg_match *match, double *partials, int32_t n, int32_t Cin,
+                                           int32_t Cout, int32_t k, int32_t stride, int32_t pad, int64_t rows_out, vmasr_stream_t stream) {
+    VMASR_REQUIRE(match, VMASR_EINVAL, "conv_mfma_fwd_match: match is required");
+    return cg_fwd(slots, n, Cin, Cout, k, stride, pad, rows_out, 1, stream, 0, match, partials);
+}
+
+VMASR_EXPORT int64_t vmasr_conv_mfma_fwd_match_partials(int32_t n, int32_t Cin, int32_t Cout, int64_t rows_out) {
+    if (n < 1 || n > CG_MATCH_SLOTS || rows_out < 1 || Cin % 128 != 0 || !vmasr_conv_mfma_supported(Cin, Cout, 1, 1)) return -1;
+    const CgConfig c = cg_config_nt(Cout, Cin, 0, true);
+    return (int64_t)n * ((rows_out + c.BM - 1) / c.BM) * (Cout / c.BN);
 }
 
 VMASR_EXPORT int vmasr_conv_f32_fwd(const vmasr_cg_slot *slots, int32_t n, int32_t Cin, int32_t Cout, int32_t k, int32_t stride,
diff --git a/vm_asr_amd/discriminator.py b/vm_asr_amd/discriminator.py
--- a/vm_asr_amd/discriminator.py
+++ b/vm_asr_amd/discriminator.py
@@ -7,7 +7,8 @@
 
 from . import _lib, knobs, mpd_ops as bind
 from .linear import linear as _linear, weight_grad as _weight_grad
-from .mpd_featloss import StackedFeatures, _FeatTapFn, _MaskedL1Fn, _masked_l1_ok, feature_loss_stacked
+from .mpd_featloss import (MatchedFeatures, StackedFeatures, _FeatTapFn, _LayerMatch, _MaskedL1Fn, _MatchedTermsFn, _masked_l1_ok,
+                           feature_loss_stacked, match_ok)
 from .mpd_layers import (_BatchedLinearFn, _BatchedLinearSplitFn, _StackedConvFirstFn, _StackedConvMfmaFn, _StackedConvPostFn,
                          _StackedConvSplitFn, _StackedIm2ColFn, _UnstackRowsFn, _bmm3, _dw3, _l1_mode, _poison, _round_up, _split_k,
                          _split_mode, scores_only, skip_weight_grads)
@@ -334,7 +335,34 @@
                 object.__setattr__(self, "_frozen", None)
         return ctx()
 
-    def _forward_batched(self, x, detach_weights=False):
+    def _match_plan(self, match, cur, n, B, cdt, tapped):
+        from . import convgemm as cg
+        if (match is None or not isinstance(match, StackedFeatures) or isinstance(match, MatchedFeatures) or not tapped or n > 8
+                or cdt != torch.float32 or not knobs.get("VMASR_MPD_FUSE_FEAT_FWD") or _lib.det_mode()):
+            return {}
+        discs = list(self.discriminators)
+        P, Hs, Cin, geo = [c.shape[1] for c in cur], [c.shape[2] for c in cur], cur[0].shape[3], []
+        stack_in = bool(knobs.get("VMASR_STACK_INPUT"))
+        for li in range(len(discs[0].layers) + 1):
+            layer = discs[0].layers[li] if li < len(discs[0].layers) else discs[0].conv_post
+            k, stride, pad, Cout = layer.kernel_size[0], layer.stride[0], layer.padding[0], layer.out_channels
+            H1 = [(h + 2 * pad - k) // stride + 1 for h in Hs]
+            Ms = tuple(B * p * h for p, h in zip(P, H1))
+            act, stacked = li < len(discs[0].layers), li > 0 and stack_in
+            path = _layer_path(li, act, cdt, cdt if li else None, stacked, k, stride, pad, Cin, Cout, n, max(Ms),
+                               max(B * p * h for p, h in zip(P, Hs)))
+            geo.append((path, stacked and path == "mfma" and Cin >= 128, Ms, _round_up(max(Ms), 256), Cin, Cout))
+            Hs, Cin = H1, Cout
+        plan = {}
+        for li, (path, pair_form, Ms, rows, Cin, Cout) in enumerate(geo):
+            if not pair_form or li >= len(match.stacks) or tuple(match.valid[li]) != Ms or not match_ok(match.stacks[li], (n, rows, Cout)):
+                continue
+            count = cg.match_partials(n, Cin, Cout, rows)
+            if count > 0:
+                plan[li] = (count, not (li + 1 < len(geo) and geo[li + 1][1]))
+        return plan
+
+    def _forward_batched(self, x, detach_weights=False, match=None):
         discs = list(self.discriminators)
         n, (B, _, T) = len(discs), x.shape
         cdt = _lib.autocast_dtype(x)
@@ -346,6 +374,10 @@
             cur.append(xp.view(B, 1, -1, p).permute(0, 3, 2, 1).to(cdt))
         fmaps, stacks, valid, taps = [[] for _ in discs], [], [], []
         next_pair = this_link = None
+        tapped = bool(x.requires_grad and torch.is_grad_enabled() and knobs.get("VMASR_FEAT_TAP"))
+        mplan = self._match_plan(match, cur, n, B, cdt, tapped)
+        mbuf = torch.empty(sum(c for c, _ in mplan.values()), dtype=torch.float64, device=x.device) if mplan else None
+        moff, mdone, n_maps = 0, {}, n * (len(discs[0].layers) + 1)
         for li in range(len(discs[0].layers) + 1):
             layers = [d.layers[li] if li < len(d.layers) else d.conv_post for d in discs]
             k, stride, pad = layers[0].kernel_size[0], layers[0].stride[0], layers[0].padding[0]
@@ -392,7 +424,15 @@
             elif path == "mfma":
                 xh, xl = pair if pair is not None else (None, None)
                 this_link = _Link()
-                y = _StackedConvMfmaFn.apply(k, stride, pad, rows, sgeom, wcache, W, bstack, src[0], xh, xl, this_link, prev_link, wpair)
+                lm = None
+                if li in mplan:
+                    if xh is None or sgeom is None or tuple(Ms) != tuple(match.valid[li]):
+                        raise RuntimeError(f"MPD: layer {li} was planned for the matching epilogue but does not read a stacked bf16 pair")
+                    count, want_y = mplan[li]
+                    lm = _LayerMatch(match.stacks[li], tuple(Ms), tuple(1.0 / (m * layers[0].out_channels * n_maps) for m in Ms),
+                                     mbuf[moff:moff + count], want_y)
+                    moff += count
+                y = _StackedConvMfmaFn.apply(k, stride, pad, rows, sgeom, wcache, W, bstack, src[0], xh, xl, this_link, prev_link, wpair, lm)
                 next_pair, this_link.pair = this_link.pair, None
             elif path == "split":
                 y = _StackedConvSplitFn.apply(k, stride, pad, rows, act, sgeom, W, bstack, *src)
@@ -407,6 +447,9 @@
                 tap = (token, t)
                 if this_link is not None:
                     this_link.tap = t
+                if path == "mfma" and lm is not None:
+                    t.offer(lm.sgn, lm.valid, lm.scale)
+                    mdone[li] = (token, t, lm.want_y)
             outs = _UnstackRowsFn.apply(y, *Ms)
             cur = [o.view(B, p, h, -1) for o, p, h in zip(outs, P, H1)]
             for f, c in zip(fmaps, cur):
@@ -414,15 +457,21 @@
             stacks.append(y)
             valid.append(tuple(Ms))
             taps.append(tap)
-        return [torch.flatten(c, 1, -1) for c in cur], StackedFeatures(fmaps, stacks, valid, taps)
+        scores = [torch.flatten(c, 1, -1) for c in cur]
+        if mplan:
+            if set(mdone) != set(mplan):
+                raise RuntimeError("MPD: a layer planned for the matching epilogue ran without its tap")
+            term = _MatchedTermsFn.apply(mbuf, tuple(t for _, t, _ in mdone.values()), *[tok for tok, _, _ in mdone.values()])
+            return scores, MatchedFeatures(fmaps, stacks, valid, taps, match, mdone.keys(), [li for li, v in mdone.items() if not v[2]], term)
+        return scores, StackedFeatures(fmaps, stacks, valid, taps)
 
     def _use_batched(self, x):
         return (x.is_cuda and not _PLAIN_OPS[0] and knobs.get("VMASR_MPD_BATCHED")
                 and len(self.discriminators) > 1)
 
-    def forward_single(self, x, detach_weights=False):
+    def forward_single(self, x, detach_weights=False, match=None):
         if self._use_batched(x):
-            return self._forward_batched(x, detach_weights)
+            return self._forward_batched(x, detach_weights, match)
         res = [d(x, detach_weights) for d in self.discriminators]
         return [r[0] for r in res], [r[1] for r in res]
 
diff --git a/vm_asr_amd/knobs.py b/vm_asr_amd/knobs.py
--- a/vm_asr_amd/knobs.py
+++ b/vm_asr_amd/knobs.py
@@ -116,6 +116,9 @@
     _k("VMASR_CONV_FIRST", "flag", 1, "the 1 -> 32 channel input convolution + GELU straight from the folded signals"),
     _k("VMASR_FEAT_TAP", "flag", 1, "a feature map's gradient (next layer's + feature-matching loss's) formed in one pass"),
     _k("VMASR_FEAT_L1", "flag", 1, "the feature-matching loss on the stacked maps in one kernel"),
+    _k("VMASR_MPD_FUSE_FEAT_FWD", "flag", 1, "the train step's fake pass forms the feature-matching term of its bf16-pair layers in their forward "
+       "epilogues against the real pass' maps (csrc/convgemm.hip EPI 3) and keeps no fp32 map that only the loss would read; 0 = finished "
+       "maps + the one-pass L1 kernel", reader="python:mpd"),
     _k("VMASR_MSD_CONV", "choice", "hip", "the MSD's strided grouped 1-D convolutions: hip = the exact-fp32 MFMA kernels (csrc/gconv1d.hip), "
        "torch = F.conv1d (A/B measurements, double backward)", values=("hip", "torch"), reader="python:msd"),
     _k("VMASR_MSD_STEM", "choice", "hip", "the MSD's 1 -> hidden stem convolution + GELU: hip = one fused pass that keeps no pre-activation "
diff --git a/vm_asr_amd/mpd_featloss.py b/vm_asr_amd/mpd_featloss.py
--- a/vm_asr_amd/mpd_featloss.py
+++ b/vm_asr_amd/mpd_featloss.py
@@ -12,6 +12,61 @@
 
     def detach(self):
         return StackedFeatures([[f.detach() for f in fs] for fs in self], [y.detach() for y in self.stacks], self.valid)
+
+
+_NO_MAP = ("MPD: layer {} of this pass has no fp32 feature map: its feature-matching term was formed in the layer's forward epilogue "
+           "against the real pass' map and nothing else reads the map (VMASR_MPD_FUSE_FEAT_FWD=0 keeps every map)")
+
+
+class _Maps(list):
+
+    def __init__(self, items, missing):
+        super().__init__(items)
+        self.missing = frozenset(missing)
+
+    def __getitem__(self, i):
+        if isinstance(i, slice):
+            return [self[j] for j in range(*i.indices(len(self)))]
+        if (i + len(self) if i < 0 else i) in self.missing:
+            raise RuntimeError(_NO_MAP.format(i + len(self) if i < 0 else i))
+        return super().__getitem__(i)
+
+    def __iter__(self):
+        return (self[i] for i in range(len(self)))
+
+
+class _LayerMatch:
+    __slots__ = ("real", "valid", "scale", "partials", "want_y", "sgn")
+
+    def __init__(self, real, valid, scale, partials, want_y):
+        self.real, self.valid, self.scale, self.partials, self.want_y, self.sgn = real, valid, scale, partials, want_y, None
+
+
+class MatchedFeatures(StackedFeatures):
+
+    def __init__(self, per_disc, stacks, valid, taps, real, matched, missing, term):
+        super().__init__([_Maps(fs, missing) for fs in per_disc], _Maps(stacks, missing), valid, taps)
+        self.real, self.matched, self.missing, self.term = real, frozenset(matched), frozenset(missing), term
+
+
+class _MatchedTermsFn(torch.autograd.Function):
+
+    @staticmethod
+    def forward(ctx, partials, taps, *tokens):
+        ctx.taps = taps
+        return partials.sum().float()
+
+    @staticmethod
+    def backward(ctx, g):
+        gtok = g.detach().reshape(1).float().contiguous()
+        for t in ctx.taps:
+            t.gtok = gtok
+        return (None, None, *([g.reshape(1)] * len(ctx.taps)))
+
+
+def match_ok(yr, shape):
+    return (torch.is_tensor(yr) and yr.is_cuda and yr.dtype == torch.float32 and yr.is_contiguous() and not yr.requires_grad
+            and tuple(yr.shape) == tuple(shape) and shape[0] <= 8 and bool(knobs.get("VMASR_FEAT_L1")))
 
 
 class _FeatTapFn(torch.autograd.Function):
@@ -74,9 +129,17 @@
 def feature_loss_stacked(real, gen):
     if not (isinstance(real, StackedFeatures) and isinstance(gen, StackedFeatures)) or real.valid != gen.valid:
         return None
+    matched = gen.matched if isinstance(gen, MatchedFeatures) else frozenset()
+    if matched and gen.real is not real:
+        raise RuntimeError("MPD: this pass was matched against other real-signal maps than the ones given (VMASR_MPD_FUSE_FEAT_FWD=0 keeps every map)")
     n_maps = sum(len(fs) for fs in gen)
     total = None
-    for yr, yg, valid, tap in zip(real.stacks, gen.stacks, real.valid, gen.taps):
+    for li, (yr, valid, tap) in enumerate(zip(real.stacks, real.valid, gen.taps)):
+        if li in matched:
+            if li == min(matched):
+                total = gen.term if total is None else total + gen.term
+            continue
+        yg = gen.stacks[li]
         R, N = min(yr.shape[1], yg.shape[1]), yg.shape[2]
         if max(valid) > R:
             return None
diff --git a/vm_asr_amd/mpd_layers.py b/vm_asr_amd/mpd_layers.py
--- a/vm_asr_amd/mpd_layers.py
+++ b/vm_asr_amd/mpd_layers.py
@@ -280,12 +280,15 @@
 class _StackedConvMfmaFn(torch.autograd.Function):
 
     @staticmethod
-    def forward(ctx, k, stride, pad, rows, geom, wcache, weight, bias, x, xh, xl, link, below=None, wpair=None):
+    def forward(ctx, k, stride, pad, rows, geom, wcache, weight, bias, x, xh, xl, link, below=None, wpair=None, match=None):
         from . import convgemm as cg
         x_req = x.requires_grad
-        x = x.float().contiguous()
+        f32 = x.shape[2] < 128 and _l1_mode() == "f32"
+        if f32 or xh is None:
+            x = x.float().contiguous()
         w = weight.detach().float().contiguous()
-        f32 = x.shape[2] < 128 and _l1_mode() == "f32"
+        if match is not None and f32:
+            raise RuntimeError("MPD: the matching forward epilogue serves the bf16-pair layers only")
         ops = wcache.get("ops") if wcache is not None else None
         if ops is None:
             ops = {} if f32 else {"w": wpair if wpair is not None else split_bf16(w)}
@@ -298,7 +301,14 @@
             if xh is None:
                 xh, xl = split_bf16(x)
             wh, wl = ops["w"]
-            pre, y, yh, yl = cg.conv_fwd(xh, xl, wh, wl, bias.detach().float().contiguous(), geom, k, stride, pad, rows, act=True)
+            b32 = bias.detach().float().contiguous()
+            if match is not None:
+                pre, y, yh, yl, match.sgn, _ = cg.conv_fwd_match(xh, xl, wh, wl, b32, geom, k, stride, pad, rows, match.real, match.valid,
+                                                                 match.scale, partials=match.partials, want_y=match.want_y)
+                if y is None:
+                    y = _poison(pre.device).expand(pre.shape)
+            else:
+                pre, y, yh, yl = cg.conv_fwd(xh, xl, wh, wl, b32, geom, k, stride, pad, rows, act=True)
         ctx.save_for_backward(xh, xl, pre, w)
         ctx.f32 = f32
         ctx.meta = (k, stride, pad, tuple(geom), ops, weight.dtype, bias.dtype, x.shape)
@@ -361,7 +371,7 @@
                 dw = cg.conv_wgrad(gh, gl, xh, xl, geom, k, stride, pad).to(wdt)
             if want_db:
                 db = db32.to(bdt)
-        return (None, None, None, None, None, None, dw, db, dx, None, None, None, None, None)
+        return (None, None, None, None, None, None, dw, db, dx, None, None, None, None, None, None)
 
 
 _POISON = {}
diff --git a/vm_asr_amd/trainer.py b/vm_asr_amd/trainer.py
--- a/vm_asr_amd/trainer.py
+++ b/vm_asr_amd/trainer.py
@@ -486,9 +486,9 @@
                 side.wait_stream(main)
                 wave_d.record_stream(side)
                 with torch.cuda.stream(side), step_amp():
-                    y_fake, f_fake = mpd.forward_single(wave_d)
+                    f_real = _detach_fmaps(f_real)
+                    y_fake, f_fake = mpd.forward_single(wave_d, match=f_real)
                     d_losses = {"mpd": self.higi_gan_loss.discriminator_loss(y_real, y_fake)}
-                    f_real = _detach_fmaps(f_real)
                     g_side = self._generator_losses(wave_d, wave_target, f_real, fake_pass=(y_fake, f_fake), parts=("mpd",))
                     total_d = sum(d_losses.values()) / acc
                     g_mpd = sum(g_side.values()) / acc if g_side else None
@@ -509,9 +509,9 @@
                     if shared:
                         mpd = unwrap(self.models["mpd"])
                         y_real, f_real = mpd.forward_single(wave_target)
-                        y_fake, f_fake = mpd.forward_single(wave_out.float())
+                        f_real = _detach_fmaps(f_real)
+                        y_fake, f_fake = mpd.forward_single(wave_out.float(), match=f_real)
                         d_losses = {"mpd": self.higi_gan_loss.discriminator_loss(y_real, y_fake)}
-                        f_real = _detach_fmaps(f_real)
                         g_losses = self._generator_losses(wave_out, wave_target, f_real, fake_pass=(y_fake, f_fake))
                     else:
                         d_losses, fmap_real = self._discriminator_losses(wave_out, wave_target)
```

New measurement: 199.5 clips/s (median of 6 runs). No clear change (+0.3%).
